# LiliMeng/network_interpretation_imagenet

Measured on NVIDIA B200. Metric: masked forward evals/sec (ResNet-101 224^2), higher is better.
Workload: dtype bf16

## Files before the change

### include/nib.h

```cpp
#ifndef NIB_H_
#define NIB_H_

#include <stddef.h>
#include <stdint.h>

#ifdef __cplusplus
extern "C" {
#endif

#define NIB_ABI_VERSION 2

enum nib_status {
  NIB_OK = 0,
  NIB_EINVAL = -1,
  NIB_ECUDA = -2,
  NIB_ENODEVICE = -3,
  NIB_ENOMEM = -4,
  NIB_ESTATE = -5,
  NIB_ENUMERIC = -6
};

int nib_abi_version(void);
const char* nib_last_error(void);
int nib_device_info(int dev, int* sm_major, int* sm_minor, int* num_sms);


enum nib_mask_mode {
  NIB_MASK_KEEP_MUL = 0,
  NIB_MASK_REMOVE_MINMAX = 1
};

enum nib_dtype { NIB_F32 = 0, NIB_BF16 = 1 };

enum nib_layout { NIB_NCHW = 0, NIB_NHWC = 1 };

typedef struct nib_mask_args {
  const float* d_img;
  const void* d_labels;
  int label_bytes;
  const uint64_t* d_sel;
  int sel_words;
  int N, C, H, W, S;
  int mode;
  const float* d_seg_minmax;
  void* d_out;
  int out_dtype;
  int layout;
  int c_stride;
  int pad_h, pad_w;
  uint8_t* d_pixel_mask;
} nib_mask_args;

int nib_segment_minmax(const float* d_img, const void* d_labels, int label_bytes,
                       int C, int H, int W, int S, float* d_seg_minmax, void* stream);

int nib_mask_synth(const nib_mask_args* args, void* stream);

int nib_mask_display_u8(const nib_mask_args* args, uint8_t* d_out, void* stream);

int nib_prep_minmax_u8(float* d_org, int C, int H, int W, uint8_t* d_u8, void* stream);


typedef struct nib_net nib_net;

enum nib_precision {
  NIB_PREC_FP32 = 0,
  NIB_PREC_BF16 = 1,
  NIB_PREC_X3 = 2,
  NIB_PREC_SPLIT = 3
};

int nib_net_create(int precision, int max_batch, nib_net** out);
int nib_net_destroy(nib_net* net);

int nib_net_add_buffer(nib_net* net, int H, int W, int C, int pad);

int nib_net_add_buffer_f32(nib_net* net, int H, int W, int C, int pad);
int nib_net_add_convert(nib_net* net, int in_buf, int out_buf);

enum nib_conv_flags {
  NIB_CONV_RELU = 1,
  NIB_CONV_PRE_BNRELU = 2
};

typedef struct nib_conv_desc {
  int in_buf, in_coff, Cin;
  int out_buf, out_coff, Cout;
  int res_buf, res_coff, res_C;
  int R, S, stride, pad;
  int flags;
} nib_conv_desc;

int nib_net_add_conv(nib_net* net, const nib_conv_desc* d, const float* h_weight,
                     const float* h_bias, const float* h_pre_scale, const float* h_pre_shift);

enum nib_pool_kind { NIB_POOL_MAX = 0, NIB_POOL_AVG = 1 };
int nib_net_add_pool(nib_net* net, int kind, int in_buf, int in_coff, int C, int out_buf,
                     int out_coff, int k, int stride, int pad,
                     const float* h_pre_scale, const float* h_pre_shift);

int nib_net_add_fc(nib_net* net, int in_buf, int Cin, int Cout, const float* h_weight,
                   const float* h_bias);

int nib_net_set_input(nib_net* net, int buf);
int nib_net_finalize(nib_net* net);

enum nib_input_layout {
  NIB_IN_NCHW_F32 = 0,
  NIB_IN_NATIVE = 1
};

int nib_net_forward(nib_net* net, const void* d_x, int x_layout, int N, float* d_logits,
                    void* stream);

int nib_net_forward_masked(nib_net* net, const nib_mask_args* args, float* d_logits, void* stream);

int nib_net_buffer_info(nib_net* net, int buf, void** d_ptr, int* H, int* W, int* C, int* pad,
                        int* dtype);
int nib_net_read_buffer_nchw(nib_net* net, int buf, int N, float* d_out, void* stream);

int nib_net_launch_counts(nib_net* net, long long* total, long long* tcgen05);
int nib_net_set_tensor_core(nib_net* net, int enable);
int nib_net_set_graph(nib_net* net, int enable);

int nib_net_profile(nib_net* net, int N, float* h_ms, int* h_kind, double* h_flops, int* h_geom,
                    int cap, int* num_ops, void* stream);

int nib_score(const float* d_logits, int N, int K, int target, int32_t* d_top1,
              float* d_target_prob, float* d_max_prob, uint8_t* d_correct, float* d_margin,
              void* stream);

int nib_score_table(const float* d_logits, int N, int K, int target, int32_t* d_top1,
                    float* d_target_prob, float* d_max_prob, uint8_t* d_correct, float* d_margin,
                    float* d_table, void* stream);

int nib_tie_compact(const float* d_margin, int N, float threshold, const uint64_t* d_sel, int words, int cap,
                    int32_t* d_idx, uint64_t* d_sel_out, int32_t* d_count, long long* d_totals, void* stream);
int nib_tie_scatter(const int32_t* d_idx, const int32_t* d_count, int cap, const int32_t* r_top1,
                    const float* r_target_prob, const float* r_max_prob, const uint8_t* r_correct,
                    int32_t* d_top1, float* d_target_prob, float* d_max_prob, uint8_t* d_correct,
                    float* d_table, void* stream);
int nib_net_set_dynamic_batch(nib_net* net, const int32_t* d_count);

typedef struct nib_comm nib_comm;
int nib_comm_unique_id(void* h_id128);
int nib_comm_init(const void* h_id128, int rank, int world, nib_comm** out);
int nib_comm_destroy(nib_comm* comm);
int nib_allgather_scores(nib_comm* comm, const float* d_local, int rows_per_rank, float* d_table, void* stream);

int nib_tc_gemm_bf16(const void* d_A, const void* d_B, float* d_C, int M, int N, int K,
                     void* stream);


int nib_gp_gram_binary(const uint64_t* d_Za, int na, const uint64_t* d_Zb, int nb, int words,
                       double length_scale, double jitter, double* d_K, int ldk, void* stream);

int nib_gp_gram_rbf(const double* d_Xa, int na, const double* d_Xb, int nb, int d,
                    double length_scale, double jitter, int same, double* d_K, int ldk,
                    void* stream);

int nib_gp_cholesky(double* d_K, int n, int ldk, int* d_info, void* stream);

int nib_gp_dgemm_sub(const double* d_A, const double* d_B, double* d_C, int M, int N, int K, void* stream);

int nib_gp_trsm(const double* d_L, int n, int ldl, double* d_B, int nrhs, int ldb, int trans,
// ... 56 lines not shown
```

### network_interpretation_imagenet_b200/_lib.py

```python
from __future__ import annotations

import ctypes as C
import os

PKG_DIR = os.path.dirname(os.path.abspath(__file__))
LIB_PATH = os.path.join(PKG_DIR, "libnib.so")

NIB_OK = 0
ABI_VERSION = 2
MASK_KEEP_MUL, MASK_REMOVE_MINMAX = 0, 1
F32, BF16 = 0, 1
NCHW, NHWC = 0, 1
PREC_FP32, PREC_BF16, PREC_X3, PREC_SPLIT = 0, 1, 2, 3
CONV_RELU, CONV_PRE_BNRELU = 1, 2
POOL_MAX, POOL_AVG = 0, 1
IN_NCHW_F32, IN_NATIVE = 0, 1


class NibError(RuntimeError):
    def __init__(self, code: int, where: str, msg: str):
        super().__init__(f"{where} failed with code {code}: {msg}")
        self.code = code


class MaskArgs(C.Structure):
    _fields_ = [
        ("d_img", C.c_void_p), ("d_labels", C.c_void_p), ("label_bytes", C.c_int),
        ("d_sel", C.c_void_p), ("sel_words", C.c_int),
        ("N", C.c_int), ("C", C.c_int), ("H", C.c_int), ("W", C.c_int), ("S", C.c_int),
        ("mode", C.c_int), ("d_seg_minmax", C.c_void_p),
        ("d_out", C.c_void_p), ("out_dtype", C.c_int), ("layout", C.c_int),
        ("c_stride", C.c_int), ("pad_h", C.c_int), ("pad_w", C.c_int),
        ("d_pixel_mask", C.c_void_p),
    ]


class ConvDesc(C.Structure):
    _fields_ = [
        ("in_buf", C.c_int), ("in_coff", C.c_int), ("Cin", C.c_int),
        ("out_buf", C.c_int), ("out_coff", C.c_int), ("Cout", C.c_int),
        ("res_buf", C.c_int), ("res_coff", C.c_int), ("res_C", C.c_int),
        ("R", C.c_int), ("S", C.c_int), ("stride", C.c_int), ("pad", C.c_int),
        ("flags", C.c_int),
    ]


_vp, _i, _d = C.c_void_p, C.c_int, C.c_double
_PROTOTYPES = {
    "nib_abi_version": (C.c_int, []),
    "nib_last_error": (C.c_char_p, []),
    "nib_device_info": (_i, [_i, C.POINTER(_i), C.POINTER(_i), C.POINTER(_i)]),
    "nib_segment_minmax": (_i, [_vp, _vp, _i, _i, _i, _i, _i, _vp, _vp]),
    "nib_mask_synth": (_i, [C.POINTER(MaskArgs), _vp]),
    "nib_mask_display_u8": (_i, [C.POINTER(MaskArgs), _vp, _vp]),
    "nib_prep_minmax_u8": (_i, [_vp, _i, _i, _i, _vp, _vp]),
    "nib_net_create": (_i, [_i, _i, C.POINTER(_vp)]),
    "nib_net_destroy": (_i, [_vp]),
    "nib_net_add_buffer": (_i, [_vp, _i, _i, _i, _i]),
    "nib_net_add_buffer_f32": (_i, [_vp, _i, _i, _i, _i]),
    "nib_net_add_convert": (_i, [_vp, _i, _i]),
    "nib_net_add_conv": (_i, [_vp, C.POINTER(ConvDesc), _vp, _vp, _vp, _vp]),
    "nib_net_add_pool": (_i, [_vp, _i, _i, _i, _i, _i, _i, _i, _i, _i, _vp, _vp]),
    "nib_net_add_fc": (_i, [_vp, _i, _i, _i, _vp, _vp]),
    "nib_net_set_input": (_i, [_vp, _i]),
    "nib_net_finalize": (_i, [_vp]),
    "nib_net_forward": (_i, [_vp, _vp, _i, _i, _vp, _vp]),
    "nib_net_forward_masked": (_i, [_vp, C.POINTER(MaskArgs), _vp, _vp]),
    "nib_net_buffer_info": (_i, [_vp, _i, C.POINTER(_vp), C.POINTER(_i), C.POINTER(_i), C.POINTER(_i),
                                 C.POINTER(_i), C.POINTER(_i)]),
    "nib_net_read_buffer_nchw": (_i, [_vp, _i, _i, _vp, _vp]),
    "nib_net_launch_counts": (_i, [_vp, C.POINTER(C.c_longlong), C.POINTER(C.c_longlong)]),
    "nib_net_set_tensor_core": (_i, [_vp, _i]),
    "nib_net_set_graph": (_i, [_vp, _i]),
    "nib_net_profile": (_i, [_vp, _i, _vp, _vp, _vp, _vp, _i, C.POINTER(_i), _vp]),
    "nib_score": (_i, [_vp, _i, _i, _i, _vp, _vp, _vp, _vp, _vp, _vp]),
    "nib_score_table": (_i, [_vp, _i, _i, _i, _vp, _vp, _vp, _vp, _vp, _vp, _vp]),
    "nib_tie_compact": (_i, [_vp, _i, C.c_float, _vp, _i, _i, _vp, _vp, _vp, _vp, _vp]),
    "nib_tie_scatter": (_i, [_vp, _vp, _i, _vp, _vp, _vp, _vp, _vp, _vp, _vp, _vp, _vp, _vp]),
    "nib_net_set_dynamic_batch": (_i, [_vp, _vp]),
    "nib_comm_unique_id": (_i, [_vp]),
    "nib_comm_init": (_i, [_vp, _i, _i, C.POINTER(_vp)]),
    "nib_comm_destroy": (_i, [_vp]),
    "nib_allgather_scores": (_i, [_vp, _vp, _i, _vp, _vp]),
    "nib_tc_gemm_bf16": (_i, [_vp, _vp, _vp, _i, _i, _i, _vp]),
    "nib_gp_gram_binary": (_i, [_vp, _i, _vp, _i, _i, _d, _d, _vp, _i, _vp]),
    "nib_gp_gram_rbf": (_i, [_vp, _i, _vp, _i, _i, _d, _d, _i, _vp, _i, _vp]),
    "nib_gp_cholesky": (_i, [_vp, _i, _i, _vp, _vp]),
    "nib_gp_trsm": (_i, [_vp, _i, _i, _vp, _i, _i, _i, _vp]),
    "nib_gp_dgemm_sub": (_i, [_vp, _vp, _vp, _i, _i, _i, _vp]),
    "nib_gp_posterior": (_i, [_vp, _i, _i, _vp, _vp, _i, _i, _d, _d, _d, _vp, _vp, _vp, _vp, _vp]),
    "nib_gp_lml": (_i, [_vp, _i, _i, _vp, _vp, C.POINTER(_d), _vp]),
    "nib_gp_lml_grad": (_i, [_vp, _vp, _vp, _vp, _i, _i, _i, _d, C.POINTER(_d), _vp]),
    "nib_gp_lml_grad_rbf": (_i, [_vp, _vp, _vp, _vp, _i, _i, _i, _d, C.POINTER(_d), _vp]),
    "nib_gp_ei": (_i, [_vp, _vp, _i, _d, _i, _vp, _vp, _vp]),
    "nib_gp_gemv_t": (_i, [_vp, _i, _i, _i, _vp, _vp, _vp]),
    "nib_gp_colsumsq": (_i, [_vp, _i, _i, _i, _vp, _vp]),
    "nib_gp_append_row": (_i, [_vp, _vp, _d, _vp, _vp, _i, _vp]),
# ... 56 lines not shown
```

### network_interpretation_imagenet_b200/classifier.py

```python
from __future__ import annotations

import ctypes as C

import numpy as np
import torch
import torch.nn as nn

from . import _lib


def _f32(t: torch.Tensor) -> np.ndarray:
    return np.ascontiguousarray(t.detach().to(torch.float32).cpu().numpy())


def fold_bn(conv_w: torch.Tensor, conv_b: torch.Tensor | None, bn: nn.BatchNorm2d | None):
    w = conv_w.detach().double()
    b = conv_b.detach().double() if conv_b is not None else torch.zeros(w.shape[0], dtype=torch.float64, device=w.device)
    if bn is not None:
        scale = bn.weight.detach().double() / torch.sqrt(bn.running_var.detach().double() + bn.eps)
        w = w * scale.view(-1, 1, 1, 1)
        b = bn.bias.detach().double() + (b - bn.running_mean.detach().double()) * scale
    elif conv_b is None:
        return w.float(), None
    return w.float(), b.float()


def bn_affine(bn: nn.BatchNorm2d):
    scale = bn.weight.detach().double() / torch.sqrt(bn.running_var.detach().double() + bn.eps)
    shift = bn.bias.detach().double() - bn.running_mean.detach().double() * scale
    return scale.float(), shift.float()


class _Builder:

    def __init__(self, precision: int, max_batch: int):
        self.lib = _lib.load()
        h = C.c_void_p()
        _lib.check(self.lib.nib_net_create(precision, max_batch, C.byref(h)), "nib_net_create")
        self.h = h
        self.shapes: dict[int, tuple[int, int, int]] = {}
        self.free: dict[tuple[int, int, int], list[int]] = {}

    def buffer(self, H, W, Cc, pad=0, pooled=True, f32=False) -> int:
        key = (H, W, Cc, bool(f32))
        if pooled and pad == 0 and self.free.get(key):
            return self.free[key].pop()
        b = (self.lib.nib_net_add_buffer_f32 if f32 else self.lib.nib_net_add_buffer)(self.h, H, W, Cc, pad)
        if b < 0:
            _lib.check(b, "nib_net_add_buffer")
        self.shapes[b] = key
        return b

    def convert(self, in_buf: int, out_buf: int):
        _lib.check(self.lib.nib_net_add_convert(self.h, in_buf, out_buf), "nib_net_add_convert")

    def release(self, b: int):
        self.free.setdefault(self.shapes[b], []).append(b)

    def conv(self, in_buf, Cin, out_buf, Cout, w, b, k, stride, pad, relu, in_coff=0, out_coff=0, res=None, res_C=0,
             pre=None):
        d = _lib.ConvDesc()
        d.in_buf, d.in_coff, d.Cin = in_buf, in_coff, Cin
        d.out_buf, d.out_coff, d.Cout = out_buf, out_coff, Cout
        d.res_buf, d.res_coff, d.res_C = (res if res is not None else -1), 0, res_C
        d.R = d.S = k
        d.stride, d.pad = stride, pad
        d.flags = (_lib.CONV_RELU if relu else 0) | (_lib.CONV_PRE_BNRELU if pre is not None else 0)
        wn = _f32(w)
        bn_ = _f32(b) if b is not None else None
        ps = _f32(pre[0]) if pre is not None else None
        pb = _f32(pre[1]) if pre is not None else None
        _lib.check(self.lib.nib_net_add_conv(self.h, C.byref(d), wn.ctypes.data,
                                             bn_.ctypes.data if bn_ is not None else None,
                                             ps.ctypes.data if ps is not None else None,
                                             pb.ctypes.data if pb is not None else None), "nib_net_add_conv")

    def pool(self, kind, in_buf, Cc, out_buf, k, stride, pad, in_coff=0, out_coff=0, pre=None):
        ps = _f32(pre[0]) if pre is not None else None
        pb = _f32(pre[1]) if pre is not None else None
        _lib.check(self.lib.nib_net_add_pool(self.h, kind, in_buf, in_coff, Cc, out_buf, out_coff, k, stride, pad,
                                             ps.ctypes.data if ps is not None else None,
                                             pb.ctypes.data if pb is not None else None), "nib_net_add_pool")

    def fc(self, in_buf, Cin, Cout, w, b):
        wn, bn_ = _f32(w), (_f32(b) if b is not None else None)
        _lib.check(self.lib.nib_net_add_fc(self.h, in_buf, Cin, Cout, wn.ctypes.data,
                                           bn_.ctypes.data if bn_ is not None else None), "nib_net_add_fc")


def _out_hw(H, k, s, p):
    return (H + 2 * p - k) // s + 1


class Classifier:

    def __init__(self, builder: _Builder, in_buf: int, in_shape, num_classes: int, precision: str, max_batch: int,
                 taps=None, arch: str = ""):
        self.lib = builder.lib
        self.h = builder.h
        self.in_buf = in_buf
        self.C, self.H, self.W = in_shape
        self.num_classes = num_classes
        self.precision = precision
        self.max_batch = max_batch
        self.taps = taps or {}
        self.arch = arch
        _lib.check(self.lib.nib_net_set_input(self.h, in_buf), "nib_net_set_input")
        _lib.check(self.lib.nib_net_finalize(self.h), "nib_net_finalize")
        ptr, H, W, Cc, pad, dt = C.c_void_p(), C.c_int(), C.c_int(), C.c_int(), C.c_int(), C.c_int()
        _lib.check(self.lib.nib_net_buffer_info(self.h, in_buf, C.byref(ptr), C.byref(H), C.byref(W), C.byref(Cc),
                                                C.byref(pad), C.byref(dt)), "nib_net_buffer_info")
        self.in_c_stride, self.in_pad = Cc.value, pad.value
        self._replicas: list["Classifier"] = []
        self._streams: list = []

    def __del__(self):
        try:
            if getattr(self, "h", None):
                self.lib.nib_net_destroy(self.h)
                self.h = None
        except Exception:
            pass

    @staticmethod
    def from_torch(module: nn.Module, input_hw=None, precision: str = "bf16", max_batch: int = 128,
                   streams: int = 1) -> "Classifier":
        c = Classifier._from_torch_one(module, input_hw, precision, max_batch)
        for _ in range(max(1, int(streams)) - 1):
            c._replicas.append(Classifier._from_torch_one(module, input_hw, precision, max_batch))
        if c._replicas:
            c._streams = [torch.cuda.Stream() for _ in range(len(c._replicas) + 1)]
        return c

    @staticmethod
    def _from_torch_one(module: nn.Module, input_hw, precision: str, max_batch: int) -> "Classifier":
        prec = {"fp32": _lib.PREC_FP32, "bf16": _lib.PREC_BF16, "x3": _lib.PREC_X3, "split": _lib.PREC_SPLIT}[precision]
        m = module.module if isinstance(module, nn.DataParallel) else module
        if hasattr(m, "layer4") and hasattr(m, "fc") and hasattr(m, "maxpool"):
            return _lower_tv_resnet(m, input_hw or (224, 224), prec, precision, max_batch)
        if _is_plain_cnn(m):
            return _lower_tv_plain(m, input_hw or (224, 224), prec, precision, max_batch)
        if precision == "split":
            raise TypeError("precision 'split' (split-bf16 tensors on the tcgen05 pair kernel) is lowered for torchvision "
                            "ResNets, VGGs and AlexNet only (every body conv needs Cin % 64 == 0 and Cout % 64 == 0); use "
                            "'x3' for this network")
        if hasattr(m, "layer3") and hasattr(m, "fc") and not hasattr(m, "layer4"):
            return _lower_resnet_cifar(m, input_hw or (32, 32), prec, precision, max_batch)
        if hasattr(m, "conv6") and hasattr(m, "fc1"):
            return _lower_mnist(m, input_hw or (28, 28), prec, precision, max_batch)
        if hasattr(m, "features") and hasattr(m, "classifier") and hasattr(m.features, "denseblock1"):
# ... 12 lines not shown

    def launch_counts(self):
        a, b = C.c_longlong(), C.c_longlong()
        _lib.check(self.lib.nib_net_launch_counts(self.h, C.byref(a), C.byref(b)), "nib_net_launch_counts")
        ra = [r.launch_counts() for r in self._replicas]
        return a.value + sum(x[0] for x in ra), b.value + sum(x[1] for x in ra)

    def _round_robin(self, N: int, launch):
        if not self._replicas:
            for i in range(0, N, self.max_batch):
                launch(self, i, min(self.max_batch, N - i))
            return
        main = torch.cuda.current_stream()
        copies = [self] + self._replicas
        used = min(len(copies), (N + self.max_batch - 1) // self.max_batch)
        for s in self._streams[:used]:
            s.wait_stream(main)
        for j, i in enumerate(range(0, N, self.max_batch)):
            k = j % len(copies)
            with torch.cuda.stream(self._streams[k]):
                launch(copies[k], i, min(self.max_batch, N - i))
        for s in self._streams[:used]:
            main.wait_stream(s)

    def forward(self, x: torch.Tensor, out: torch.Tensor | None = None) -> torch.Tensor:
        if not x.is_cuda:
            raise RuntimeError("Classifier.forward needs a CUDA tensor: this engine has no CPU path")
        x = x.to(torch.float32).contiguous()
        N = int(x.shape[0])
        if tuple(x.shape[1:]) != (self.C, self.H, self.W):
            raise ValueError(f"input {tuple(x.shape)} does not match network input {(self.C, self.H, self.W)}")
        if out is None:
            out = torch.empty(N, self.num_classes, dtype=torch.float32, device=x.device)

        def launch(c, i, n):
            _lib.check(c.lib.nib_net_forward(c.h, x[i:i + n].data_ptr(), _lib.IN_NCHW_F32, n,
                                             out[i:i + n].data_ptr(), _lib.stream_handle()), "nib_net_forward")

        self._round_robin(N, launch)
        return out

    def forward_masked(self, synth, sel_bits, mode: int, out: torch.Tensor | None = None) -> torch.Tensor:
        d_sel = synth.device_bits(sel_bits)
        N = int(d_sel.shape[0])
        if out is None:
            out = torch.empty(N, self.num_classes, dtype=torch.float32, device=d_sel.device)
        if mode == _lib.MASK_REMOVE_MINMAX:
            synth.seg_minmax()

        def launch(c, i, n):
            a = synth.mask_args(d_sel[i:i + n], mode, None, 0, 0)
            _lib.check(c.lib.nib_net_forward_masked(c.h, C.byref(a), out[i:i + n].data_ptr(), _lib.stream_handle()),
                       "nib_net_forward_masked")

        self._round_robin(N, launch)
        return out

    def profile(self, N: int):
        cap = 4096
        ms = (C.c_float * cap)()
        kind = (C.c_int * cap)()
        flops = (C.c_double * cap)()
        geom = (C.c_int * (8 * cap))()
        n = C.c_int()
        _lib.check(self.lib.nib_net_profile(self.h, N, ms, kind, flops, geom, cap, C.byref(n), _lib.stream_handle()),
                   "nib_net_profile")
        return [(ms[i], kind[i], flops[i], tuple(geom[8 * i:8 * i + 8])) for i in range(n.value)]

    def read_tap(self, name: str, N: int) -> torch.Tensor:
        buf = self.taps[name]
        H, W, Cc = C.c_int(), C.c_int(), C.c_int()
        _lib.check(self.lib.nib_net_buffer_info(self.h, buf, None, C.byref(H), C.byref(W), C.byref(Cc), None, None),
                   "nib_net_buffer_info")
        out = torch.empty(N, Cc.value, H.value, W.value, dtype=torch.float32, device="cuda")
        _lib.check(self.lib.nib_net_read_buffer_nchw(self.h, buf, N, out.data_ptr(), _lib.stream_handle()),
                   "nib_net_read_buffer_nchw")
        return out


def _in_cpad(Cin: int) -> int:
    return 4 if Cin <= 4 else Cin


def _lower_tv_resnet(m, hw, prec, precision, max_batch):
    H, W = hw
    b = _Builder(prec, max_batch)
    cin = m.conv1.in_channels
    c1 = m.conv1
    stem_tc = (precision == "bf16" and c1.kernel_size == (7, 7) and c1.stride == (2, 2) and c1.padding == (3, 3) and cin <= 8)
    split = precision == "split"
    x_in = (b.buffer(H, W, 4 if cin <= 4 else 8, pad=3, pooled=False) if stem_tc
            else b.buffer(H, W, _in_cpad(cin), pooled=False, f32=split))
    Hc, Wc = _out_hw(H, c1.kernel_size[0], c1.stride[0], c1.padding[0]), _out_hw(W, c1.kernel_size[0], c1.stride[0], c1.padding[0])
    t = b.buffer(Hc, Wc, c1.out_channels, f32=split)
    w, bias = fold_bn(c1.weight, c1.bias, m.bn1)
    b.conv(x_in, cin, t, c1.out_channels, w, bias, c1.kernel_size[0], c1.stride[0], c1.padding[0], relu=True)
    mp = m.maxpool
    k, s, p = mp.kernel_size, mp.stride, mp.padding
    Hp, Wp = _out_hw(Hc, k, s, p), _out_hw(Wc, k, s, p)
    x = b.buffer(Hp, Wp, c1.out_channels, f32=split)
    b.pool(_lib.POOL_MAX, t, c1.out_channels, x, k, s, p)
    b.release(t)
    if split:
        xs = b.buffer(Hp, Wp, c1.out_channels)
        b.convert(x, xs)
        b.release(x)
        x = xs
    Cx, Hx, Wx = c1.out_channels, Hp, Wp
    for layer in (m.layer1, m.layer2, m.layer3, m.layer4):
        for blk in layer:
            convs = [(blk.conv1, blk.bn1), (blk.conv2, blk.bn2)]
            if hasattr(blk, "conv3"):
                convs.append((blk.conv3, blk.bn3))
            if blk.downsample is not None:
                dc, dbn = blk.downsample[0], blk.downsample[1]
                Hd, Wd = _out_hw(Hx, dc.kernel_size[0], dc.stride[0], dc.padding[0]), _out_hw(Wx, dc.kernel_size[0], dc.stride[0], dc.padding[0])
                idn = b.buffer(Hd, Wd, dc.out_channels)
                w, bias = fold_bn(dc.weight, dc.bias, dbn)
                b.conv(x, Cx, idn, dc.out_channels, w, bias, dc.kernel_size[0], dc.stride[0], dc.padding[0], relu=False)
            else:
                idn = x
            cur, Cc, Hh, Ww = x, Cx, Hx, Wx
            tmp = []
            for i, (cv, bn) in enumerate(convs):
                last = i == len(convs) - 1
                Ho, Wo = _out_hw(Hh, cv.kernel_size[0], cv.stride[0], cv.padding[0]), _out_hw(Ww, cv.kernel_size[0], cv.stride[0], cv.padding[0])
                o = b.buffer(Ho, Wo, cv.out_channels)
                w, bias = fold_bn(cv.weight, cv.bias, bn)
                if last:
                    b.conv(cur, Cc, o, cv.out_channels, w, bias, cv.kernel_size[0], cv.stride[0], cv.padding[0],
                           relu=True, res=idn, res_C=cv.out_channels)
                else:
                    b.conv(cur, Cc, o, cv.out_channels, w, bias, cv.kernel_size[0], cv.stride[0], cv.padding[0], relu=True)
                    tmp.append(o)
                cur, Cc, Hh, Ww = o, cv.out_channels, Ho, Wo
            for tbuf in tmp:
                b.release(tbuf)
            if idn != x:
                b.release(idn)
            b.release(x)
            x, Cx, Hx, Wx = cur, Cc, Hh, Ww
    if split:
        xf = b.buffer(Hx, Wx, Cx, f32=True)
        b.convert(x, xf)
        x = xf
    feat = b.buffer(1, 1, Cx, f32=split)
    assert Hx == Wx, "global average pool expects a square map"
    b.pool(_lib.POOL_AVG, x, Cx, feat, Hx, Hx, 0)
    b.fc(feat, Cx, m.fc.out_features, m.fc.weight, m.fc.bias)
    return Classifier(b, x_in, (cin, H, W), m.fc.out_features, precision, max_batch, arch="tv_resnet")


def _lower_resnet_cifar(m, hw, prec, precision, max_batch):
    H, W = hw
    b = _Builder(prec, max_batch)
    cp = (lambda c: max(c, 64)) if precision == "bf16" else (lambda c: c)

    def padw(w, bias, co, ci):
        if co == w.shape[0] and ci == w.shape[1]:
            return w, bias
        wp = torch.zeros(co, ci, w.shape[2], w.shape[3], dtype=w.dtype, device=w.device)
        wp[:w.shape[0], :w.shape[1]] = w
        bp = None
        if bias is not None:
            bp = torch.zeros(co, dtype=bias.dtype, device=bias.device)
            bp[:bias.shape[0]] = bias
        return wp, bp

    x_in = b.buffer(H, W, _in_cpad(3), pooled=False)
    x = b.buffer(H, W, cp(16))
    w, bias = padw(*fold_bn(m.conv1.weight, None, m.bn1), cp(16), 3)
    b.conv(x_in, 3, x, cp(16), w, bias, 3, 1, 1, relu=True)
    Cx, Hx, Wx = 16, H, W
    for layer in (m.layer1, m.layer2, m.layer3):
        for blk in layer:
            s = blk.conv1.stride[0]
            planes = blk.conv1.out_channels
            Ho, Wo = _out_hw(Hx, 3, s, 1), _out_hw(Wx, 3, s, 1)
            t = b.buffer(Ho, Wo, cp(planes))
            w, bias = padw(*fold_bn(blk.conv1.weight, None, blk.bn1), cp(planes), cp(Cx))
            b.conv(x, cp(Cx), t, cp(planes), w, bias, 3, s, 1, relu=True)
            if blk.downsample is not None:
                ks = blk.downsample.avg.kernel_size
                ks = ks if isinstance(ks, int) else ks[0]
                idn = b.buffer(_out_hw(Hx, ks, ks, 0), _out_hw(Wx, ks, ks, 0), cp(Cx))
                b.pool(_lib.POOL_AVG, x, cp(Cx), idn, ks, ks, 0)
            else:
                idn = x
            o = b.buffer(Ho, Wo, cp(planes))
            w, bias = padw(*fold_bn(blk.conv2.weight, None, blk.bn2), cp(planes), cp(planes))
            b.conv(t, cp(planes), o, cp(planes), w, bias, 3, 1, 1, relu=True, res=idn, res_C=cp(Cx))
            b.release(t)
            if idn != x:
                b.release(idn)
            b.release(x)
            x, Cx, Hx, Wx = o, planes, Ho, Wo
    ks = m.avgpool.kernel_size
    ks = ks if isinstance(ks, int) else ks[0]
    assert _out_hw(Hx, ks, ks, 0) == 1, "AvgPool2d(8) must reduce to 1x1 (models/resnet.py:103)"
    feat = b.buffer(1, 1, cp(Cx))
    b.pool(_lib.POOL_AVG, x, cp(Cx), feat, ks, ks, 0)
    fw = m.fc.weight
    if cp(Cx) != Cx:
        fw = torch.zeros(fw.shape[0], cp(Cx), dtype=fw.dtype, device=fw.device)
        fw[:, :Cx] = m.fc.weight
    b.fc(feat, cp(Cx), m.fc.out_features, fw, m.fc.bias)
    return Classifier(b, x_in, (3, H, W), m.fc.out_features, precision, max_batch, arch="resnet_cifar")


def _lower_mnist(m, hw, prec, precision, max_batch):
    H, W = hw
    b = _Builder(prec, max_batch)
    x_in = b.buffer(H, W, _in_cpad(1), pooled=False)
    cur, Cc, Hh, Ww = x_in, 1, H, W
    taps = {}
    for name in ("conv1", "conv2", "conv3", "conv4", "conv5"):
        seq = getattr(m, name)
        cv, bn = seq[0], seq[1]
        Ho, Wo = _out_hw(Hh, 3, cv.stride[0], cv.padding[0]), _out_hw(Ww, 3, cv.stride[0], cv.padding[0])
        o = b.buffer(Ho, Wo, cv.out_channels, pooled=False)
        w, bias = fold_bn(cv.weight, cv.bias, bn)
        b.conv(cur, Cc, o, cv.out_channels, w, bias, 3, cv.stride[0], cv.padding[0], relu=True)
        cur, Cc, Hh, Ww = o, cv.out_channels, Ho, Wo
        if name == "conv2":
            taps["x0"] = o
        if name == "conv4":
            taps["x1"] = o
    cv = m.conv6
    o = b.buffer(Hh, Ww, cv.out_channels, pooled=False)
    b.conv(cur, Cc, o, cv.out_channels, cv.weight.detach().float(), cv.bias.detach().float(), 3, 1, 1, relu=False)
    taps["x2"] = o
    feat = b.buffer(1, 1, cv.out_channels)
    assert Hh == Ww
    b.pool(_lib.POOL_AVG, o, cv.out_channels, feat, Hh, Hh, 0)
    b.fc(feat, cv.out_channels, m.fc1.out_features, m.fc1.weight, m.fc1.bias)
    return Classifier(b, x_in, (1, H, W), m.fc1.out_features, precision, max_batch, taps=taps, arch="mnist")


def _dense_block(b: _Builder, layers, blk_buf, C0, H, W, Ctot):
    cur = C0
    for lyr in layers:
        n1, c1 = lyr.norm1, lyr.conv1
        has_bottleneck = hasattr(lyr, "conv2") and getattr(lyr, "conv2") is not None
        if has_bottleneck:
            n2, c2 = lyr.norm2, lyr.conv2
            mid = b.buffer(H, W, c1.out_channels)
            w, bias = fold_bn(c1.weight, None, n2)
            b.conv(blk_buf, cur, mid, c1.out_channels, w, bias, 1, 1, 0, relu=True, pre=bn_affine(n1))
            b.conv(mid, c1.out_channels, blk_buf, c2.out_channels, c2.weight.detach().float(), None, 3, 1, 1,
                   relu=False, out_coff=cur)
            b.release(mid)
            cur += c2.out_channels
        else:
            b.conv(blk_buf, cur, blk_buf, c1.out_channels, c1.weight.detach().float(), None, 3, 1, 1, relu=False,
                   out_coff=cur, pre=bn_affine(n1))
            cur += c1.out_channels
    assert cur == Ctot
    return cur


def _lower_tv_densenet(m, hw, prec, precision, max_batch):
    H, W = hw
    f = m.features
    b = _Builder(prec, max_batch)
    c0 = f.conv0
    stem_tc = (precision == "bf16" and c0.kernel_size == (7, 7) and c0.stride == (2, 2) and c0.padding == (3, 3))
    x_in = b.buffer(H, W, 4, pad=3, pooled=False) if stem_tc else b.buffer(H, W, _in_cpad(3), pooled=False)
    Hc, Wc = _out_hw(H, 7, 2, 3), _out_hw(W, 7, 2, 3)
    t = b.buffer(Hc, Wc, c0.out_channels)
    w, bias = fold_bn(c0.weight, None, f.norm0)
    b.conv(x_in, 3, t, c0.out_channels, w, bias, 7, 2, 3, relu=True)
    Hx, Wx = _out_hw(Hc, 3, 2, 1), _out_hw(Wc, 3, 2, 1)
    blocks = [getattr(f, n) for n in ("denseblock1", "denseblock2", "denseblock3", "denseblock4")]
    trans = [getattr(f, n) for n in ("transition1", "transition2", "transition3")]
    Cin = c0.out_channels
    prev, prev_is_stem = t, True
    for bi, blk in enumerate(blocks):
        layers = list(blk.children())
        growth = layers[0].conv2.out_channels
        Ctot = Cin + growth * len(layers)
        buf = b.buffer(Hx, Wx, Ctot, pooled=False)
        if prev_is_stem:
            b.pool(_lib.POOL_MAX, prev, Cin, buf, 3, 2, 1)
            b.release(prev)
        else:
            b.pool(_lib.POOL_AVG, prev, Cin, buf, 2, 2, 0)
            b.release(prev)
        _dense_block(b, layers, buf, Cin, Hx, Wx, Ctot)
        if bi < len(trans):
            tr = trans[bi]
            Co = tr.conv.out_channels
            tt = b.buffer(Hx, Wx, Co)
            b.conv(buf, Ctot, tt, Co, tr.conv.weight.detach().float(), None, 1, 1, 0, relu=False, pre=bn_affine(tr.norm))
            prev, prev_is_stem = tt, False
            Cin = Co
            Hx, Wx = Hx // 2, Wx // 2
        else:
            feat = b.buffer(1, 1, Ctot)
            assert Hx == Wx
            b.pool(_lib.POOL_AVG, buf, Ctot, feat, Hx, Hx, 0, pre=bn_affine(f.norm5))
            b.fc(feat, Ctot, m.classifier.out_features, m.classifier.weight, m.classifier.bias)
    return Classifier(b, x_in, (3, H, W), m.classifier.out_features, precision, max_batch, arch="tv_densenet")


def _lower_densenet_cifar(m, hw, prec, precision, max_batch):
    H, W = hw
    b = _Builder(prec, max_batch)
    x_in = b.buffer(H, W, _in_cpad(3), pooled=False)
    seq = list(m.blocks.children())
    Cin = m.stem.out_channels
    Hx, Wx = H, W
    prev = None
    for i in range(0, len(seq), 2):
        layers = list(seq[i].children())
        growth = (layers[0].conv2 if hasattr(layers[0], "conv2") else layers[0].conv1).out_channels
        Ctot = Cin + growth * len(layers)
        buf = b.buffer(Hx, Wx, Ctot, pooled=False)
        if prev is None:
            b.conv(x_in, 3, buf, Cin, m.stem.weight.detach().float(), None, 3, 1, 1, relu=False)
        else:
            b.pool(_lib.POOL_AVG, prev, Cin, buf, 2, 2, 0)
            b.release(prev)
        _dense_block(b, layers, buf, Cin, Hx, Wx, Ctot)
        if i + 1 < len(seq):
            tr = list(seq[i + 1].children())
            Co = tr[2].out_channels
            tt = b.buffer(Hx, Wx, Co)
            b.conv(buf, Ctot, tt, Co, tr[2].weight.detach().float(), None, 1, 1, 0, relu=False, pre=bn_affine(tr[0]))
            prev, Cin = tt, Co
            Hx, Wx = Hx // 2, Wx // 2
        else:
            feat = b.buffer(1, 1, Ctot)
            assert Hx == 8 and Wx == 8, "avg_pool2d(8) expects an 8x8 map (models/densenet.py:96)"
            b.pool(_lib.POOL_AVG, buf, Ctot, feat, 8, 8, 0, pre=bn_affine(m.norm5))
            b.fc(feat, Ctot, m.classifier.out_features, m.classifier.weight, m.classifier.bias)
    return Classifier(b, x_in, (3, H, W), m.classifier.out_features, precision, max_batch, arch="densenet_cifar")


def _is_plain_cnn(m) -> bool:
    return (isinstance(getattr(m, "features", None), nn.Sequential) and isinstance(getattr(m, "classifier", None), nn.Sequential)
            and not hasattr(m.features, "denseblock1"))


def _pair(v):
    return tuple(v) if isinstance(v, (tuple, list)) else (v, v)


def _plain_cnn_layers(m, hw, precision):
    H, W = hw
    C = None
    ops = []
    mods = list(m.features.children())
    i = 0
    while i < len(mods):
        mod = mods[i]
        if isinstance(mod, nn.Conv2d):
            k, s, p, d = _pair(mod.kernel_size), _pair(mod.stride), _pair(mod.padding), _pair(mod.dilation)
            if (mod.groups != 1 or d != (1, 1) or k[0] != k[1] or s[0] != s[1] or isinstance(mod.padding, str) or p[0] != p[1]
                    or mod.padding_mode != "zeros"):
                raise TypeError(f"unsupported Conv2d in features[{i}]: {mod} (needs groups 1, dilation 1, square kernel, "
                                "stride and zero padding)")
            if C is not None and mod.in_channels != C:
                raise TypeError(f"features[{i}]: {mod} takes {mod.in_channels} channels, the map has {C}")
            bn = None
            if i + 1 < len(mods) and isinstance(mods[i + 1], nn.BatchNorm2d):
# ... 121 lines not shown
```

### network_interpretation_imagenet_b200/csrc/conv_tc.cu

```cuda
#include "common.cuh"
#include "layers.cuh"
#include <cuda.h>
#include <string.h>
#include <stdlib.h>

namespace nib {

static constexpr int TC_BLOCK_M = 128;
static constexpr int TC_BLOCK_K = 64;
static constexpr int TC_UMMA_K = 16;
static constexpr int TC_THREADS = 192;

struct TcKernelParams {
  const float* bias;
  const __nv_bfloat16* res;
  void* out;
  int M;
  int Cout;
  int out_cstride, out_coff;
  int res_cstride, res_coff;
  int relu;
  int out_f32;
  int num_k_blocks;
  int cblocks;
// ... 412 lines not shown
                                             int c2, int c3) {
  asm volatile(
      "cp.async.bulk.tensor.4d.cta_group::2.shared::cluster.global.mbarrier::complete_tx::bytes [%0], [%1, {%3, %4, %5, %6}], [%2];"
      ::"r"(dst), "l"(reinterpret_cast<uint64_t>(tm)), "r"(leader_bar), "r"(c0), "r"(c1), "r"(c2), "r"(c3)
      : "memory");
}
__device__ __forceinline__ void tma2_load_5d(uint32_t dst, const CUtensorMap* tm, uint32_t leader_bar, int c0, int c1,
                                             int c2, int c3, int c4) {
  asm volatile(
      "cp.async.bulk.tensor.5d.cta_group::2.shared::cluster.global.mbarrier::complete_tx::bytes [%0], [%1, {%3, %4, %5, %6, %7}], [%2];"
      ::"r"(dst), "l"(reinterpret_cast<uint64_t>(tm)), "r"(leader_bar), "r"(c0), "r"(c1), "r"(c2), "r"(c3), "r"(c4)
      : "memory");
}
__device__ __forceinline__ void tma2_load_im2col_4d(uint32_t dst, const CUtensorMap* tm, uint32_t leader_bar, int c,
                                                    int w, int h, int n, uint16_t off_w, uint16_t off_h) {
  asm volatile(
      "cp.async.bulk.tensor.4d.im2col.cta_group::2.shared::cluster.global.mbarrier::complete_tx::bytes"
      " [%0], [%1, {%3, %4, %5, %6}], [%2], {%7, %8};"
      ::"r"(dst), "l"(reinterpret_cast<uint64_t>(tm)), "r"(leader_bar), "r"(c), "r"(w), "r"(h), "r"(n), "h"(off_w),
      "h"(off_h)
      : "memory");
}
__device__ __forceinline__ bool elect_one() {
  uint32_t pred;
  asm volatile(
      "{\n\t.reg .pred p;\n\t"
      "elect.sync _|p, 0xffffffff;\n\t"
      "selp.u32 %0, 1, 0, p;\n\t}"
      : "=r"(pred));
  return pred != 0;
}
__device__ __forceinline__ void named_bar_sync(int id, int nthreads) {
  asm volatile("bar.sync %0, %1;" ::"r"(id), "r"(nthreads) : "memory");
}

__device__ __forceinline__ void tmem_ld_32x32b_x64(uint32_t taddr, uint32_t (&v)[64]) {
  asm volatile(
      "tcgen05.ld.sync.aligned.32x32b.x64.b32 "
      "{%0, %1, %2, %3, %4, %5, %6, %7, %8, %9, %10, %11, %12, %13, %14, %15, "
      "%16, %17, %18, %19, %20, %21, %22, %23, %24, %25, %26, %27, %28, %29, %30, %31, "
      "%32, %33, %34, %35, %36, %37, %38, %39, %40, %41, %42, %43, %44, %45, %46, %47, "
      "%48, %49, %50, %51, %52, %53, %54, %55, %56, %57, %58, %59, %60, %61, %62, %63}, [%64];"
      : "=r"(v[0]), "=r"(v[1]), "=r"(v[2]), "=r"(v[3]), "=r"(v[4]), "=r"(v[5]), "=r"(v[6]), "=r"(v[7]),
        "=r"(v[8]), "=r"(v[9]), "=r"(v[10]), "=r"(v[11]), "=r"(v[12]), "=r"(v[13]), "=r"(v[14]), "=r"(v[15]),
        "=r"(v[16]), "=r"(v[17]), "=r"(v[18]), "=r"(v[19]), "=r"(v[20]), "=r"(v[21]), "=r"(v[22]), "=r"(v[23]),
        "=r"(v[24]), "=r"(v[25]), "=r"(v[26]), "=r"(v[27]), "=r"(v[28]), "=r"(v[29]), "=r"(v[30]), "=r"(v[31]),
        "=r"(v[32]), "=r"(v[33]), "=r"(v[34]), "=r"(v[35]), "=r"(v[36]), "=r"(v[37]), "=r"(v[38]), "=r"(v[39]),
        "=r"(v[40]), "=r"(v[41]), "=r"(v[42]), "=r"(v[43]), "=r"(v[44]), "=r"(v[45]), "=r"(v[46]), "=r"(v[47]),
        "=r"(v[48]), "=r"(v[49]), "=r"(v[50]), "=r"(v[51]), "=r"(v[52]), "=r"(v[53]), "=r"(v[54]), "=r"(v[55]),
        "=r"(v[56]), "=r"(v[57]), "=r"(v[58]), "=r"(v[59]), "=r"(v[60]), "=r"(v[61]), "=r"(v[62]), "=r"(v[63])
      : "r"(taddr)
      : "memory");
}
__device__ __forceinline__ uint64_t pack_f32x2(uint32_t lo, uint32_t hi) {
  uint64_t r;
  asm("mov.b64 %0, {%1, %2};" : "=l"(r) : "r"(lo), "r"(hi));
  return r;
}
__device__ __forceinline__ uint64_t add_f32x2(uint64_t a, uint64_t b) {
  uint64_t r;
  asm("add.rn.f32x2 %0, %1, %2;" : "=l"(r) : "l"(a), "l"(b));
  return r;
}
__device__ __forceinline__ uint32_t cvt_bf16x2(uint64_t a) {
  uint32_t lo, hi, r;
  asm("mov.b64 {%0, %1}, %2;" : "=r"(lo), "=r"(hi) : "l"(a));
  asm("cvt.rn.bf16x2.f32 %0, %1, %2;" : "=r"(r) : "f"(__uint_as_float(hi)), "f"(__uint_as_float(lo)));
  return r;
}
__device__ __forceinline__ uint32_t max_bf16x2(uint32_t a, uint32_t b) {
  uint32_t r;
  asm("max.NaN.bf16x2 %0, %1, %2;" : "=r"(r) : "r"(a), "r"(b));
  return r;
}
__device__ __forceinline__ void mbar_arrive_remote(uint32_t cluster_addr) {
  asm volatile("mbarrier.arrive.shared::cluster.b64 _, [%0];" ::"r"(cluster_addr) : "memory");
}

template <int BLOCK_N>
__host__ __device__ constexpr uint32_t make_idesc_bf16_pair() {
  return (1u << 4) | (1u << 7) | (1u << 10) | ((uint32_t)(BLOCK_N >> 3) << 17) | ((uint32_t)(256 >> 4) << 24);
}

template <int BLOCK_N, int STAGES, bool HAS_RES, bool BRES, bool SPLIT = false>
__global__ void __cluster_dims__(2, 1, 1) __launch_bounds__(TC3_THREADS_XF, 1)
conv_tc3_kernel(const __grid_constant__ CUtensorMap tmA, const __grid_constant__ CUtensorMap tmB,
                const __grid_constant__ CUtensorMap tmOut, const __grid_constant__ CUtensorMap tmOutTail,
                const __grid_constant__ CUtensorMap tmRes, const TcKernelParams p) {
  using SM = Tc3Smem<BLOCK_N, STAGES, HAS_RES, BRES, SPLIT>;
  extern __shared__ __align__(1024) uint8_t smem_raw[];
  const uint32_t smem_base = smem_u32(smem_raw);
  if ((smem_base & 1023u) != 0) {
    if (threadIdx.x == 0 && p.err_flag) atomicExch(p.err_flag, 9u);
    __trap();
  }
  const uint32_t bar_base = smem_base + SM::BAR_OFFSET;
  auto full_bar = [&](int s) { return bar_base + 8u * s; };
  auto empty_bar = [&](int s) { return bar_base + 8u * (STAGES + s); };
  auto tmem_full_bar = [&](int b) { return bar_base + 8u * (2 * STAGES + b); };
  auto tmem_empty_bar = [&](int b) { return bar_base + 8u * (2 * STAGES + 2 + b); };
  auto res_full_bar = [&](int b) { return bar_base + 8u * (2 * STAGES + 4 + b); };
  auto box_free_bar = [&](int b) { return bar_base + 8u * (2 * STAGES + 4 + SM::NBUF + b); };
  const uint32_t bres_full_bar = bar_base + 8u * (2 * STAGES + 4 + 2 * SM::NBUF);
  auto afull_bar = [&](int s) { return bar_base + 8u * (2 * STAGES + 5 + 2 * SM::NBUF + s); };
  auto xf_bar = [&](int s) { return bar_base + 8u * (3 * STAGES + 5 + 2 * SM::NBUF + s); };
  const bool xform = !BRES && !SPLIT && p.xf_scale != nullptr;
  const uint32_t tmem_slot = bar_base + 8u * SM::NUM_BARS;
  uint32_t* tmem_slot_ptr = reinterpret_cast<uint32_t*>(smem_raw + (tmem_slot - smem_u32(smem_raw)));
  auto box_addr = [&](int buf) { return smem_base + SM::BOX_OFFSET + (uint32_t)buf * SM::BOX_BYTES; };

  const int warp = threadIdx.x >> 5;
  const int lane = threadIdx.x & 31;
  const uint32_t rank = cluster_ctarank();
  const int pair = blockIdx.x >> 1;
  const int npairs = gridDim.x >> 1;
  int m_tiles_live = p.m_tiles;
  if (SPLIT && p.dyn_n != nullptr) {
    const long long live = (long long)max(*p.dyn_n, 0) * p.P * p.Q;
    const int t = (int)((live + p.tile_rows - 1) / p.tile_rows);
    if (t < m_tiles_live) m_tiles_live = t;
  }
  const int m_pairs = (m_tiles_live + 1) >> 1;
  const int total_tiles = m_pairs * p.n_tiles;
  constexpr uint32_t TMEM_COLS = 2 * BLOCK_N;
  const bool dbg_on = p.dbg != nullptr;
  long long t_acc[4] = {0, 0, 0, 0};
  long long t_loop0 = 0;
  if (dbg_on && threadIdx.x == 0) {
    unsigned long long gt;
    asm volatile("mov.u64 %0, %%globaltimer;" : "=l"(gt));
    p.dbg[(size_t)blockIdx.x * 16 + 12] = gt;
    p.dbg[(size_t)blockIdx.x * 16 + 14] = (unsigned long long)clock64();
  }
#define TC3_TIMED(slot, stmt)                                      \
  do {                                                             \
    if (dbg_on) { const long long _t = clock64(); stmt; t_acc[slot] += clock64() - _t; } \
    else { stmt; }                                                 \
  } while (0)

  if (warp == 0 && lane == 0) {
    prefetch_tmap(&tmA);
    prefetch_tmap(&tmB);
    prefetch_tmap(&tmOut);
    if (HAS_RES) prefetch_tmap(&tmRes);
    for (int s = 0; s < STAGES; ++s) {
      mbar_init(full_bar(s), 1);
      mbar_init(empty_bar(s), 1);
    }
    for (int b = 0; b < 2; ++b) {
      mbar_init(tmem_full_bar(b), 1);
      mbar_init(tmem_empty_bar(b), SM::EMPTY_ARRIVALS);
    }
    for (int b = 0; b < SM::NBUF; ++b) {
      mbar_init(res_full_bar(b), 1);
      mbar_init(box_free_bar(b), 4);
    }
    mbar_init(bres_full_bar, 1);
    for (int s2 = 0; s2 < STAGES; ++s2) {
      mbar_init(afull_bar(s2), 1);
      mbar_init(xf_bar(s2), 2 * TC3_XF_WARPS);
    }
    asm volatile("fence.mbarrier_init.release.cluster;" ::: "memory");
  }
  if (warp == 1) {
    asm volatile("tcgen05.alloc.cta_group::2.sync.aligned.shared::cta.b32 [%0], %1;" ::"r"(tmem_slot), "r"(TMEM_COLS) : "memory");
    asm volatile("tcgen05.relinquish_alloc_permit.cta_group::2.sync.aligned;" ::: "memory");
// ... 110 lines not shown
          const int ca = SPLIT ? (cb >= p.a_wrap ? cb - p.a_wrap : cb) : cb;
          const int c0 = ca * TC_BLOCK_K + p.in_coff;
          if (p.im2col == 1) {
            tma2_load_im2col_4d(a_dst, &tmA, lbar, c0, w0, h0, img, (uint16_t)tap_s, (uint16_t)tap_r);
          } else if (p.im2col == 2) {
            tma2_load_4d(a_dst, &tmA, lbar, 0, 0, h0 + kb, img);
          } else if (p.im2col == 3) {
            tma2_load_4d(a_dst, &tmA, lbar, 0, 0, h0 + 2 * kb, img);
            tma2_load_4d(a_dst + SM::A_BYTES / 2, &tmA, lbar, 0, 0, h0 + 2 * kb + 1, img);
          } else if (xform) {
            mbar_arrive_expect_tx(afull_bar(stage), (uint32_t)p.a_bytes);
            tma_load_2d(a_dst, &tmA, afull_bar(stage), c0, m0);
          } else {
            tma2_load_2d(a_dst, &tmA, lbar, c0, m0);
          }
          if (!BRES) tma2_load_2d(a_dst + SM::A_BYTES, &tmB, lbar, kb * TC_BLOCK_K, n0 + b_row0);
        }
        __syncwarp();
        if (++stage == STAGES) { stage = 0; phase ^= 1u; }
        ++kb;
        if (++cb == p.cblocks) { cb = 0; if (++tap_s == p.S) { tap_s = 0; ++tap_r; } }
      }
      if (HAS_RES) {
        issue_pending(true);
        pend_b = 0;
        pend_set = it % SM::RSETS;
        pend_par = (uint32_t)((it / SM::RSETS) & 1);
        pend_m0 = m0;
        pend_n0 = n0;
      }
    }
    if (HAS_RES) issue_pending(true);
    if (dbg_on && lane == 0) {
      unsigned long long* d = p.dbg + (size_t)blockIdx.x * 16;
      d[0] = (unsigned long long)t_acc[0]; d[1] = (unsigned long long)t_acc[1];
      d[8] = (unsigned long long)(clock64() - t_loop0);
    }
  } else if (warp == 1) {
    if (rank == 0) {
      constexpr uint32_t idesc = make_idesc_bf16_pair<BLOCK_N>();
      int stage = 0;
      uint32_t phase = 0;
      int it = 0;
      if (dbg_on) t_loop0 = clock64();
      if (BRES) mbar_wait(bres_full_bar, 0, p.err_flag, 7);
      for (int tile = pair; tile < total_tiles; tile += npairs, ++it) {
        const int ab = it & 1;
        TC3_TIMED(1, mbar_wait(tmem_empty_bar(ab), (uint32_t)(((it >> 1) & 1) ^ 1), p.err_flag, 5));
        tc_fence_after();
        const uint32_t d_tmem = tmem_base + (uint32_t)(ab * BLOCK_N);
        if (BRES && !HAS_RES && p.im2col == 4) {
          const int npb = 4 / p.halo_cb, pbuf = it % npb;
          const int st4 = 2 * p.halo_cb * pbuf;
          TC3_TIMED(0, mbar_wait(full_bar(st4), (uint32_t)((it / npb) & 1), p.err_flag, 2));
          tc_fence_after();
          if (elect_one()) {
            const uint32_t patch = smem_base + st4 * SM::STAGE_BYTES;
            const uint32_t bhb = (uint32_t)(p.halo_n * 64);
            const uint32_t idesc_h = p.halo_n == 32 ? make_idesc_bf16_pair<32>() : idesc;
#pragma unroll 1
            for (int kb = 0; kb < 9 * p.halo_cb; ++kb) {
              const int tap = p.halo_cb == 2 ? (kb >> 1) : kb, c = p.halo_cb == 2 ? (kb & 1) : 0;
              const int dy = tap / 3, dx = tap - 3 * dy;
              const uint32_t a_addr = patch + (uint32_t)(2 * c) * SM::STAGE_BYTES + (uint32_t)(dy * p.halo_wp + dx) * 128u;
              const uint64_t adesc = make_smem_desc_sw128(a_addr);
              const uint64_t bdesc = make_smem_desc_sw128(smem_base + SM::BRES_OFFSET + (uint32_t)kb * bhb);
#pragma unroll
              for (int k = 0; k < TC_BLOCK_K / TC_UMMA_K; ++k)
                umma2_bf16(d_tmem, adesc + (uint64_t)(2 * k), bdesc + (uint64_t)(2 * k), idesc_h, (kb | k) != 0);
            }
            umma2_commit_both(empty_bar(st4));
            umma2_commit_both(tmem_full_bar(ab));
          }
          __syncwarp();
          continue;
        }
        if (BRES && !HAS_RES && p.im2col == 5) {
          TC3_TIMED(0, mbar_wait(full_bar(stage), phase, p.err_flag, 2));
          tc_fence_after();
          if (elect_one()) {
            const int q0 = ((tile / p.n_tiles) % p.col_tiles) * p.tile_rows;
            const uint32_t a_addr = smem_base + stage * SM::STAGE_BYTES + 16u * (uint32_t)q0;
            const uint32_t lbo = p.halo_swap ? 128u : 16u, sbo = p.halo_swap ? 16u : 128u;
#pragma unroll 1
            for (int r = 0; r < p.raw_rows; ++r) {
              const uint32_t b_addr = smem_base + SM::BRES_OFFSET + (r >> 1) * SM::BH_BYTES + (r & 1) * (SM::BH_BYTES / 2);
#pragma unroll
              for (int ks = 0; ks < 2; ++ks) {
                const uint64_t adesc = make_smem_desc_nosw(a_addr + (uint32_t)(r * p.halo_wp) + ks * 32, lbo, sbo);
                const uint64_t bdesc = make_smem_desc_sw64(b_addr + ks * 32);
                umma2_bf16(d_tmem, adesc, bdesc, idesc, (r | ks) != 0);
              }
            }
            umma2_commit_both(empty_bar(stage));
            umma2_commit_both(tmem_full_bar(ab));
          }
          __syncwarp();
          if (++stage == STAGES) { stage = 0; phase ^= 1u; }
          continue;
        }
        for (int kk = 0; kk < p.num_k_blocks; ++kk) {
          const int kb = kk;
          TC3_TIMED(0, mbar_wait(full_bar(stage), phase, p.err_flag, 2));
          if (xform) TC3_TIMED(0, mbar_wait(xf_bar(stage), phase, p.err_flag, 8));
          tc_fence_after();
          if (elect_one()) {
            const uint32_t a_addr = smem_base + stage * SM::STAGE_BYTES;
            const uint32_t b_addr = BRES ? smem_base + SM::BRES_OFFSET + kb * SM::BH_BYTES : a_addr + SM::A_BYTES;
            if (BRES && p.im2col == 3) {
#pragma unroll
              for (int k = 0; k < TC_BLOCK_K / TC_UMMA_K; ++k) {
                const uint64_t adesc = make_smem_desc_sw64(a_addr + (k >> 1) * (SM::A_BYTES / 2) + (k & 1) * 32);
                const uint64_t bdesc = make_smem_desc_sw64(b_addr + (k >> 1) * (SM::BH_BYTES / 2) + (k & 1) * 32);
                umma2_bf16(d_tmem, adesc, bdesc, idesc, (kk | k) != 0);
              }
            } else {
              const uint64_t adesc = make_smem_desc_sw128(a_addr);
              const uint64_t bdesc = make_smem_desc_sw128(b_addr);
#pragma unroll
              for (int k = 0; k < TC_BLOCK_K / TC_UMMA_K; ++k)
                umma2_bf16(d_tmem, adesc + (uint64_t)(2 * k), bdesc + (uint64_t)(2 * k), idesc, (kk | k) != 0);
            }
            umma2_commit_both(empty_bar(stage));
            if (kk == p.num_k_blocks - 1) umma2_commit_both(tmem_full_bar(ab));
          }
          __syncwarp();
          if (++stage == STAGES) { stage = 0; phase ^= 1u; }
        }
      }
      if (dbg_on && lane == 0) {
        unsigned long long* d = p.dbg + (size_t)blockIdx.x * 16;
        d[2] = (unsigned long long)t_acc[0]; d[3] = (unsigned long long)t_acc[1];
        d[9] = (unsigned long long)(clock64() - t_loop0);
      }
    }
  } else if (warp >= 2 + 8) {
    if (xform) {
      const int t = (int)threadIdx.x - 32 * (2 + 8);
      const int cl = t & 7, rb = t >> 3;
      const uint32_t lead_xf0 = mapa_shared(xf_bar(0), 0);
      int stage = 0;
      uint32_t phase = 0;
      for (int tile = pair; tile < total_tiles; tile += npairs) {
        for (int kk = 0; kk < p.num_k_blocks; ++kk) {
          const float4 s0 = __ldg(reinterpret_cast<const float4*>(p.xf_scale + kk * TC_BLOCK_K + 8 * cl));
          const float4 s1 = __ldg(reinterpret_cast<const float4*>(p.xf_scale + kk * TC_BLOCK_K + 8 * cl + 4));
          const float4 h0 = __ldg(reinterpret_cast<const float4*>(p.xf_shift + kk * TC_BLOCK_K + 8 * cl));
          const float4 h1 = __ldg(reinterpret_cast<const float4*>(p.xf_shift + kk * TC_BLOCK_K + 8 * cl + 4));
          mbar_wait(afull_bar(stage), phase, p.err_flag, 9);
          const uint32_t a_addr = smem_base + stage * SM::STAGE_BYTES;
#pragma unroll
          for (int i = 0; i < 8; ++i) {
            const int r = rb + 16 * i;
            const uint32_t addr = a_addr + (uint32_t)r * 128u + ((uint32_t)(cl ^ (r & 7)) << 4);
            const uint4 raw = lds_v4(addr);
            const __nv_bfloat162* v = reinterpret_cast<const __nv_bfloat162*>(&raw);
            const float2 a = __bfloat1622float2(v[0]), b = __bfloat1622float2(v[1]), c = __bfloat1622float2(v[2]), d = __bfloat1622float2(v[3]);
            uint4 o;
            __nv_bfloat162 q;
            q = __floats2bfloat162_rn(fmaxf(fmaf(a.x, s0.x, h0.x), 0.f), fmaxf(fmaf(a.y, s0.y, h0.y), 0.f)); o.x = *reinterpret_cast<uint32_t*>(&q);
            q = __floats2bfloat162_rn(fmaxf(fmaf(b.x, s0.z, h0.z), 0.f), fmaxf(fmaf(b.y, s0.w, h0.w), 0.f)); o.y = *reinterpret_cast<uint32_t*>(&q);
            q = __floats2bfloat162_rn(fmaxf(fmaf(c.x, s1.x, h1.x), 0.f), fmaxf(fmaf(c.y, s1.y, h1.y), 0.f)); o.z = *reinterpret_cast<uint32_t*>(&q);
            q = __floats2bfloat162_rn(fmaxf(fmaf(d.x, s1.z, h1.z), 0.f), fmaxf(fmaf(d.y, s1.w, h1.w), 0.f)); o.w = *reinterpret_cast<uint32_t*>(&q);
            sts_v4(addr, o);
          }
          fence_async_smem();
          __syncwarp();
          if (lane == 0) mbar_arrive_remote(lead_xf0 + 8u * stage);
          if (++stage == STAGES) { stage = 0; phase ^= 1u; }
        }
      }
    }
  } else {
    const int ew = warp - 2;
    const int g = ew >> 2;
    const int quarter = warp & 3;
// ... 141 lines not shown
          uint64_t a2 = pack_f32x2(v[c * 8 + 4], v[c * 8 + 5]), a3 = pack_f32x2(v[c * 8 + 6], v[c * 8 + 7]);
          if (has_bias) {
            const uint4 b0 = lds_v4(bsrc + (uint32_t)(c * 32)), b1 = lds_v4(bsrc + (uint32_t)(c * 32 + 16));
            a0 = add_f32x2(a0, pack_f32x2(b0.x, b0.y)); a1 = add_f32x2(a1, pack_f32x2(b0.z, b0.w));
            a2 = add_f32x2(a2, pack_f32x2(b1.x, b1.y)); a3 = add_f32x2(a3, pack_f32x2(b1.z, b1.w));
          }
          if (HAS_RES) {
            const uint4 r = lds_v4(obase + ((((uint32_t)c) ^ sw) << 4));
            a0 = add_f32x2(a0, pack_f32x2(r.x << 16, r.x & 0xFFFF0000u)); a1 = add_f32x2(a1, pack_f32x2(r.y << 16, r.y & 0xFFFF0000u));
            a2 = add_f32x2(a2, pack_f32x2(r.z << 16, r.z & 0xFFFF0000u)); a3 = add_f32x2(a3, pack_f32x2(r.w << 16, r.w & 0xFFFF0000u));
          }
          o[c * 4 + 0] = max_bf16x2(cvt_bf16x2(a0), relu_floor); o[c * 4 + 1] = max_bf16x2(cvt_bf16x2(a1), relu_floor);
          o[c * 4 + 2] = max_bf16x2(cvt_bf16x2(a2), relu_floor); o[c * 4 + 3] = max_bf16x2(cvt_bf16x2(a3), relu_floor);
        }
        if (halo) {
          if (quarter == 0 && lane == 0) TC3_TIMED(2, bulk_wait_read<0>());
          TC3_TIMED(3, named_bar_sync(1 + g, 128));
          if (halo_valid) {
#pragma unroll
            for (int c = 0; c < 8; ++c)
              if (c < 4 || p.halo_n == 64)
                sts_v4(halo_base + ((((uint32_t)c) ^ halo_sw) << 4), make_uint4(o[c * 4], o[c * 4 + 1], o[c * 4 + 2], o[c * 4 + 3]));
          }
          fence_async_smem();
          TC3_TIMED(3, named_bar_sync(1 + g, 128));
          if (quarter == 0 && lane == 0) {
            tma_store_2d(&tmOutTail, box_addr(g), p.out_coff + n0, m0);
            bulk_commit();
          }
          continue;
        }
        if (!HAS_RES) {
          if (lane == 0) TC3_TIMED(2, bulk_wait_read<0>());
          __syncwarp();
        }
#pragma unroll
        for (int c = 0; c < 8; ++c)
          sts_v4(obase + ((((uint32_t)c) ^ sw) << 4), make_uint4(o[c * 4], o[c * 4 + 1], o[c * 4 + 2], o[c * 4 + 3]));
        fence_async_smem();
        __syncwarp();
        if (lane == 0) {
          if (rows_here >= 32) tma_store_2d(&tmOut, slab, p.out_coff + n0 + b * 64, m0 + quarter * 32);
          else if (rows_here > 0) tma_store_2d(&tmOutTail, slab, p.out_coff + n0 + b * 64, m0 + quarter * 32);
          bulk_commit();
          if (HAS_RES) {
            if (u > 0) {
              TC3_TIMED(2, bulk_wait_read<1>());
              mbar_arrive(box_free_bar(buf - 1));
            }
            if (u == SM::UNITS - 1) {
              TC3_TIMED(2, bulk_wait_read<0>());
              mbar_arrive(box_free_bar(buf));
            }
          }
        }
      }
    }
    if (lane == 0) bulk_wait_read<0>();
    if (dbg_on && warp == 2 && lane == 0) {
      unsigned long long* d = p.dbg + (size_t)blockIdx.x * 16;
      d[4] = (unsigned long long)t_acc[0]; d[5] = (unsigned long long)t_acc[1];
      d[6] = (unsigned long long)t_acc[2]; d[7] = (unsigned long long)t_acc[3];
      d[10] = (unsigned long long)(clock64() - t_loop0);
      d[11] = (unsigned long long)lt;
    }
    tc_fence_before();
  }
#undef TC3_TIMED
  __syncthreads();
  cluster_sync_all();
  if (warp == 1) {
    tc_fence_after();
    asm volatile("tcgen05.dealloc.cta_group::2.sync.aligned.b32 %0, %1;" ::"r"(tmem_base), "r"(TMEM_COLS) : "memory");
  }
  if (dbg_on && threadIdx.x == 0) {
    unsigned long long gt;
    asm volatile("mov.u64 %0, %%globaltimer;" : "=l"(gt));
    p.dbg[(size_t)blockIdx.x * 16 + 13] = gt;
    p.dbg[(size_t)blockIdx.x * 16 + 15] = (unsigned long long)clock64();
  }
}


struct TcFusedParams {
  const float* bias1;
  const float* bias2;
  const __nv_bfloat16* res;
  int M, m_tiles;
  int kb1;
  int nch;
  int n1;
  int relu1, relu2;
  unsigned int* err_flag;
  unsigned long long* dbg;
};

template <int N2>
struct TcFusedSmem {
  static constexpr int S1 = 4, S2 = 4;
  static constexpr int A1_BYTES = TC_BLOCK_M * TC_BLOCK_K * 2;
  static constexpr int A1_KB = 4;
  static constexpr int B1_BYTES = 64 * TC_BLOCK_K * 2;
  static constexpr int B2_BYTES = (N2 / 2) * TC_BLOCK_K * 2;
  static constexpr int BOX_BYTES = TC_BLOCK_M * 128;
  static constexpr int R1_OFFSET = A1_KB * A1_BYTES;
  static constexpr int R2_OFFSET = R1_OFFSET + S1 * B1_BYTES;
  static constexpr int STG_OFFSET = R2_OFFSET + S2 * B2_BYTES;
  static constexpr int BIAS1_OFFSET = STG_OFFSET + 4 * BOX_BYTES;
  static constexpr int BIAS2_OFFSET = BIAS1_OFFSET + 2 * 128 * 4;
  static constexpr int BAR_OFFSET = BIAS2_OFFSET + N2 * 4;
  static constexpr int NUM_BARS = 2 * S1 + 2 * S2 + 14;
  static constexpr int TOTAL = BAR_OFFSET + NUM_BARS * 8 + 16;
  static constexpr int EP2_WARPS = N2 / 16;
};

static constexpr int TCF_THREADS = 64 + 512;
template <int N2>
__global__ void __cluster_dims__(2, 1, 1) __launch_bounds__(TCF_THREADS, 1)
conv_fused_ca_kernel(const __grid_constant__ CUtensorMap tmA1, const __grid_constant__ CUtensorMap tmB1,
                     const __grid_constant__ CUtensorMap tmRes, const __grid_constant__ CUtensorMap tmY,
                     const __grid_constant__ CUtensorMap tmB2, const __grid_constant__ CUtensorMap tmOut2,
                     const TcFusedParams p) {
  using SM = TcFusedSmem<N2>;
  constexpr int S1 = SM::S1, S2 = SM::S2;
  extern __shared__ __align__(1024) uint8_t smem_raw[];
  const uint32_t smem_base = smem_u32(smem_raw);
  if ((smem_base & 1023u) != 0) {
    if (threadIdx.x == 0 && p.err_flag) atomicExch(p.err_flag, 9u);
    __trap();
  }
  const uint32_t bar_base = smem_base + SM::BAR_OFFSET;
  auto full1 = [&](int s) { return bar_base + 8u * s; };
  auto empty1 = [&](int s) { return bar_base + 8u * (S1 + s); };
  auto full2 = [&](int s) { return bar_base + 8u * (2 * S1 + s); };
  auto empty2 = [&](int s) { return bar_base + 8u * (2 * S1 + S2 + s); };
  const uint32_t bar2 = bar_base + 8u * (2 * S1 + 2 * S2);
  auto acc1_full = [&](int b) { return bar2 + 8u * b; };
  auto acc1_empty = [&](int b) { return bar2 + 8u * (2 + b); };
  auto res_full = [&](int b) { return bar2 + 8u * (4 + b); };
  auto y_ready = [&](int b) { return bar2 + 8u * (6 + b); };
  auto stage_free = [&](int b) { return bar2 + 8u * (8 + b); };
  const uint32_t acc2_full = bar2 + 8u * 10;
  const uint32_t acc2_empty = bar2 + 8u * 11;
  const uint32_t a1_full = bar2 + 8u * 12;
  const uint32_t a1_empty = bar2 + 8u * 13;
  const uint32_t tmem_slot = bar_base + 8u * SM::NUM_BARS;
  uint32_t* tmem_slot_ptr = reinterpret_cast<uint32_t*>(smem_raw + (tmem_slot - smem_base));
  auto stg = [&](int set, int box) { return smem_base + SM::STG_OFFSET + (uint32_t)(set * 2 + box) * SM::BOX_BYTES; };
  float* bias1_s = reinterpret_cast<float*>(smem_raw + SM::BIAS1_OFFSET);
  float* bias2_s = reinterpret_cast<float*>(smem_raw + SM::BIAS2_OFFSET);

  const int warp = threadIdx.x >> 5;
  const int lane = threadIdx.x & 31;
  const uint32_t rank = cluster_ctarank();
  const int pair = blockIdx.x >> 1;
  const int npairs = gridDim.x >> 1;
  const int m_pairs = (p.m_tiles + 1) >> 1;
  constexpr uint32_t TMEM_COLS = 512;
  constexpr uint32_t ACC2_COL = 256;

  if (warp == 0 && lane == 0) {
    prefetch_tmap(&tmA1); prefetch_tmap(&tmB1); prefetch_tmap(&tmRes);
    prefetch_tmap(&tmY); prefetch_tmap(&tmB2); prefetch_tmap(&tmOut2);
    for (int s = 0; s < S1; ++s) { mbar_init(full1(s), 1); mbar_init(empty1(s), 1); }
    for (int s = 0; s < S2; ++s) { mbar_init(full2(s), 1); mbar_init(empty2(s), 1); }
    for (int b = 0; b < 2; ++b) {
// ... 233 lines not shown
          }
          __syncwarp();
          if (j + 2 < p.nch) fetch_residual(use + 1u, j + 2, m0);
          else if (more_tiles) fetch_residual(use + 1u, g, m0_next);
        }
      }
      if (ep2) {
        FT(3, mbar_wait(acc2_full, (uint32_t)it & 1u, p.err_flag, 31));
        tc_fence_after();
        if (lane == 0) bulk_wait_read<0>();
        __syncwarp();
        const int col2 = G * 64;
        drain32(lane_taddr + ACC2_COL + (uint32_t)col2, bias2_s + col2, 0, false, relu2_floor);
        drain32(lane_taddr + ACC2_COL + (uint32_t)(col2 + 32), bias2_s + col2 + 32, 4, false, relu2_floor);
        tc_fence_before();
        __syncwarp();
        if (lane == 0) mbar_arrive_remote(lead_acc2_empty);
        fence_async_smem();
        __syncwarp();
        if (lane == 0) {
          tma_store_2d(&tmOut2, slab, col2, m0 + quarter * 32);
          bulk_commit();
          bulk_wait_read<0>();
          mbar_arrive(stage_free(g));
        }
        __syncwarp();
      }
      if (ep2 && more_tiles) fetch_residual((uint32_t)((it * p.nch + (p.nch - 2 + g)) >> 1) + 1u, g, m0_next);
    }
    if (lane == 0) bulk_wait_read<0>();
    tc_fence_before();
  }
#undef FT
  if (dbg_on && lane == 0 && (warp == 0 || warp == 1 || warp == 4 || warp == 8)) {
    const int role = warp == 0 ? 0 : warp == 1 ? 1 : warp == 4 ? 2 : 3;
    unsigned long long* d = p.dbg + (size_t)blockIdx.x * 32 + role * 8;
    for (int i = 0; i < 7; ++i) d[i] = (unsigned long long)t_acc[i];
    d[7] = (unsigned long long)(clock64() - t_role0);
  }
  __syncthreads();
  cluster_sync_all();
  if (warp == 1) {
    tc_fence_after();
    asm volatile("tcgen05.dealloc.cta_group::2.sync.aligned.b32 %0, %1;" ::"r"(tmem_base), "r"(TMEM_COLS) : "memory");
  }
}

typedef CUresult (*PFN_encodeTiled)(CUtensorMap*, CUtensorMapDataType, cuuint32_t, void*, const cuuint64_t*,
                                    const cuuint64_t*, const cuuint32_t*, const cuuint32_t*, CUtensorMapInterleave,
                                    CUtensorMapSwizzle, CUtensorMapL2promotion, CUtensorMapFloatOOBfill);
typedef CUresult (*PFN_encodeIm2col)(CUtensorMap*, CUtensorMapDataType, cuuint32_t, void*, const cuuint64_t*,
                                     const cuuint64_t*, const int*, const int*, cuuint32_t, cuuint32_t,
                                     const cuuint32_t*, CUtensorMapInterleave, CUtensorMapSwizzle,
                                     CUtensorMapL2promotion, CUtensorMapFloatOOBfill);
static PFN_encodeTiled g_encodeTiled = nullptr;
static PFN_encodeIm2col g_encodeIm2col = nullptr;

static int load_driver_fns() {
  if (g_encodeTiled && g_encodeIm2col) return NIB_OK;
  cudaDriverEntryPointQueryResult q;
  void* fn = nullptr;
  NIB_CUDA(cudaGetDriverEntryPoint("cuTensorMapEncodeTiled", &fn, cudaEnableDefault, &q));
  if (q != cudaDriverEntryPointSuccess || !fn) { set_error("cuTensorMapEncodeTiled not available"); return NIB_ECUDA; }
  g_encodeTiled = (PFN_encodeTiled)fn;
  fn = nullptr;
  NIB_CUDA(cudaGetDriverEntryPoint("cuTensorMapEncodeIm2col", &fn, cudaEnableDefault, &q));
  if (q != cudaDriverEntryPointSuccess || !fn) { set_error("cuTensorMapEncodeIm2col not available"); return NIB_ECUDA; }
  g_encodeIm2col = (PFN_encodeIm2col)fn;
  return NIB_OK;
}

struct TcConvPlan {
  CUtensorMap tmA, tmB, tmOut, tmRes;
  CUtensorMap tmBh;
  CUtensorMap tmOut32, tmOutTail;
  int v3;
  int split;
  int block_n, stages;
  int im2col;
  int tile_rows;
  int num_k_blocks, cblocks;
  int halo_wp, halo_r, halo_tpi, halo_cb, halo_n;
  int raw_rows, col_tiles;
  unsigned int* err_flag;
};

static unsigned int* g_err_flag = nullptr;

static int encode_2d_bf16(CUtensorMap* tm, const void* ptr, uint64_t inner, uint64_t outer, uint64_t row_bytes,
                          uint32_t box_inner, uint32_t box_outer) {
  cuuint64_t dims[2] = {inner, outer};
  cuuint64_t strides[1] = {row_bytes};
  cuuint32_t box[2] = {box_inner, box_outer};
  cuuint32_t es[2] = {1, 1};
  CUresult r = g_encodeTiled(tm, CU_TENSOR_MAP_DATA_TYPE_BFLOAT16, 2, const_cast<void*>(ptr), dims, strides, box, es,
                             CU_TENSOR_MAP_INTERLEAVE_NONE, CU_TENSOR_MAP_SWIZZLE_128B,
                             CU_TENSOR_MAP_L2_PROMOTION_L2_256B, CU_TENSOR_MAP_FLOAT_OOB_FILL_NONE);
  if (r != CUDA_SUCCESS) {
    set_error("cuTensorMapEncodeTiled failed (%d): dims=(%llu,%llu) row_bytes=%llu box=(%u,%u) ptr=%p", (int)r,
              (unsigned long long)inner, (unsigned long long)outer, (unsigned long long)row_bytes, box_inner,
              box_outer, ptr);
    return NIB_ECUDA;
  }
  return NIB_OK;
}

bool tc_conv_is_stem(const ConvParams& p) {
  return p.R == 7 && p.S == 7 && p.stride == 2 && p.pad == 3 && p.Cin <= 8 && p.in_cstride == 8 && p.in_coff == 0 &&
         p.in_halo == 3 && p.Cout % 32 == 0 && p.Q <= TC_BLOCK_M && p.out_halo == 0 && p.out_cstride % 8 == 0 &&
         p.out_coff % 8 == 0 && p.pre_scale == nullptr && p.res == nullptr && p.w_alt != nullptr &&
         (p.Win + 2 * p.in_halo) >= 2 * (p.Q - 1) + 8;
}

bool tc_conv_is_stem4(const ConvParams& p) {
  return p.R == 7 && p.S == 7 && p.stride == 2 && p.pad == 3 && p.Cin <= 4 && p.in_cstride == 4 &&
         p.in_coff == 0 && p.in_halo == 3 && p.Cout % 64 == 0 && p.Q <= TC_BLOCK_M && p.out_halo == 0 &&
         p.out_cstride % 8 == 0 && p.out_coff % 8 == 0 && p.pre_scale == nullptr && p.res == nullptr &&
         p.w_alt != nullptr && (p.Win + 2 * p.in_halo) % 2 == 0 && (p.Win + 2 * p.in_halo) >= 2 * (p.Q - 1) + 8 &&
         (p.Hin + 2 * p.in_halo) >= 2 * (p.P - 1) + 8;
}

static int raw_row_inner(int row_el) {
  for (int c = 256; c >= 8; c -= 8)
    if (row_el % c == 0 && row_el / c <= 256) return c;
  return 0;
}

static int raw3x3_col_tiles(int Q) {
  if (Q <= TC_BLOCK_M) return 1;
  for (int t = 2; Q / t >= TC_BLOCK_M / 2; ++t)
    if (Q % t == 0 && Q / t <= TC_BLOCK_M) return t;
  return 0;
}

bool tc_conv_is_raw3x3(const ConvParams& p) {
  static const bool off = getenv("NIB_TC_NO_HALO") != nullptr;
  if (off || p.split) return false;
  if (!(p.R == 3 && p.S == 3 && p.stride == 1 && p.pad == 1 && p.Cin <= 8 && p.in_cstride == 8 && p.in_coff == 0 &&
        p.in_halo == 1))
    return false;
  if (!(p.Cout == 64 || p.Cout == 128) || p.out_halo != 0 || p.out_cstride % 8 != 0 || p.out_coff % 8 != 0) return false;
  if (p.pre_scale != nullptr || p.res != nullptr || p.w_alt == nullptr || p.P != p.Hin || p.Q != p.Win) return false;
  const int t = raw3x3_col_tiles(p.Q);
  if (t == 0) return false;
  const int Wp = p.Win + 2, row_bytes = Wp * 16;
  if (3 * row_bytes + 16 > TC_BLOCK_M * TC_BLOCK_K * 2) return false;
  if (2 * row_bytes + 16 * (p.Q - p.Q / t + TC_BLOCK_M - 1) + 64 > TC_BLOCK_M * TC_BLOCK_K * 2) return false;
  return raw_row_inner(Wp * 8) > 0;
}

static int halo_rows_per_tile(int H, int Wp) {
  for (int r = TC_BLOCK_M / Wp; r >= 1; --r)
    if (H % r == 0) return r;
  return 0;
}
bool tc_conv_is_halo3x3(const ConvParams& p) {
  static const bool off = getenv("NIB_TC_NO_HALO") != nullptr;
  if (off || p.split) return false;
  if (!(p.R == 3 && p.S == 3 && p.stride == 1 && p.pad == 1)) return false;
  if (!((p.Cin == 64 && (p.Cout == 64 || p.Cout == 32)) || (p.Cin == 128 && p.Cout == 32))) return false;
  if (p.res != nullptr || p.pre_scale != nullptr || p.in_halo != 0 || p.out_halo != 0) return false;
  if (p.in_cstride % 8 != 0 || p.in_coff % 8 != 0 || p.out_cstride % 8 != 0 || p.out_coff % 8 != 0) return false;
  if (p.P != p.Hin || p.Q != p.Win) return false;
  const int Wp = p.Win + 2;
  if (Wp > 63) return false;
  const int R = halo_rows_per_tile(p.Hin, Wp);
  return R >= 1 && R * Wp >= 56;
}

bool tc_conv_supported(const ConvParams& p) {
  if (p.split) {
    if (p.Cin % TC_BLOCK_K != 0 || p.Cout % 64 != 0 || p.in_coff != 0 || p.out_coff != 0 || p.in_lo_off != p.Cin) return false;
    if (p.in_cstride != 2 * p.Cin || p.out_cstride < p.out_lo_off + p.Cout || p.out_lo_off % 64 != 0) return false;
    if (p.in_halo != 0 || p.out_halo != 0 || p.pre_scale != nullptr || p.R != p.S || p.pad > 127 || p.R > 16) return false;
    if (p.res != nullptr && (p.res_C != p.Cout || p.res_coff != 0 || p.res_lo_off % 64 != 0 || p.res_cstride < p.res_lo_off + p.Cout))
      return false;
    return true;
  }
  if (tc_conv_is_stem(p) || tc_conv_is_stem4(p) || tc_conv_is_raw3x3(p)) return true;
  if (p.Cin % TC_BLOCK_K != 0) return false;
  if (p.in_cstride % 8 != 0 || p.in_coff % 8 != 0) return false;
  if (p.Cout % 32 != 0) return false;
  if (p.out_cstride % 8 != 0 || p.out_coff % 8 != 0) return false;
  if (p.in_halo != 0 || p.out_halo != 0) return false;
  if (p.pre_scale != nullptr && !(p.pre_padded && p.R == 1 && p.S == 1 && p.stride == 1 && p.pad == 0 && p.Cout % 64 == 0 &&
                                  p.res == nullptr))
    return false;
  if (p.res != nullptr && (p.res_C != p.Cout || p.res_cstride % 8 != 0 || p.res_coff % 8 != 0)) return false;
  if (p.R != p.S) return false;
  if (p.pad > 127 || p.R > 16) return false;
  return true;
}

static int pick_block_n(int Cout) {
  if (Cout % 256 == 0) return 256;
  if (Cout % 128 == 0) return 128;
  if (Cout % 64 == 0) return 64;
  return 32;
}

static int finish_plan(TcConvPlan* plan, const ConvParams& p, int max_batch, const void* w_ptr, int K) {
  plan->v3 = 0;
  static const bool v1_only = getenv("NIB_TC_V1") != nullptr;
  if (v1_only) return NIB_OK;
  const bool bn_ok = plan->block_n == 64 || plan->block_n == 128 || plan->block_n == 256;
  if (!bn_ok || p.Cout % plan->block_n != 0) return NIB_OK;
  const uint64_t rows = (uint64_t)max_batch * p.P * p.Q;
  int rc = encode_2d_bf16(&plan->tmOut, p.out, (uint64_t)p.out_cstride, rows, (uint64_t)p.out_cstride * 2, 64,
                          (uint32_t)plan->tile_rows);
  if (rc != NIB_OK) return rc;
  if (p.res != nullptr) {
    rc = encode_2d_bf16(&plan->tmRes, p.res, (uint64_t)p.res_cstride, rows, (uint64_t)p.res_cstride * 2, 64, TC_BLOCK_M);
    if (rc != NIB_OK) return rc;
  } else {
    plan->tmRes = plan->tmOut;
  }
  rc = encode_2d_bf16(&plan->tmBh, w_ptr, (uint64_t)K, (uint64_t)p.Cout, (uint64_t)K * 2, TC_BLOCK_K,
                      (uint32_t)(plan->block_n / 2));
  if (rc != NIB_OK) return rc;
  rc = encode_2d_bf16(&plan->tmOut32, p.out, (uint64_t)p.out_cstride, rows, (uint64_t)p.out_cstride * 2, 64, 32);
  if (rc != NIB_OK) return rc;
  const int tail = plan->tile_rows % 32;
  rc = encode_2d_bf16(&plan->tmOutTail, p.out, (uint64_t)p.out_cstride, rows, (uint64_t)p.out_cstride * 2, 64,
                      (uint32_t)(tail ? tail : 32));
  if (rc != NIB_OK) return rc;
  plan->v3 = 1;
  return NIB_OK;
}

int tc_conv_plan_create(const ConvParams& p, int max_batch, TcConvPlan** out) {
  int rc = load_driver_fns();
  if (rc != NIB_OK) return rc;
  if (!g_err_flag) {
    NIB_CUDA(cudaMalloc(&g_err_flag, sizeof(unsigned int)));
    NIB_CUDA(cudaMemset(g_err_flag, 0, sizeof(unsigned int)));
  }
  TcConvPlan* plan = new TcConvPlan();
  memset(plan, 0, sizeof(*plan));
  plan->err_flag = g_err_flag;
  plan->block_n = pick_block_n(p.Cout);
  plan->tile_rows = TC_BLOCK_M;
  if (tc_conv_is_stem4(p)) {
    plan->im2col = 3;
    plan->cblocks = 1;
    plan->num_k_blocks = 4;
    plan->tile_rows = p.Q;
    const int Hp = p.Hin + 6, Wp = p.Win + 6;
    int inner = 0;
    {
      static const bool off = getenv("NIB_TC_NO_HALO") != nullptr;
      if (!off && 6 * Wp * 8 + 16 * 127 + 64 <= 16384) inner = raw_row_inner(Wp * 4);
    }
    if (inner > 0) {
      plan->im2col = 5;
      plan->raw_rows = 7;
      plan->col_tiles = 1;
      plan->halo_wp = Wp * 8;
      cuuint64_t dims[4] = {(cuuint64_t)inner, (cuuint64_t)(Wp * 4 / inner), (cuuint64_t)Hp, (cuuint64_t)max_batch};
      cuuint64_t strides[3] = {(cuuint64_t)inner * 2, (cuuint64_t)Wp * 8, (cuuint64_t)Hp * Wp * 8};
      cuuint32_t box[4] = {(cuuint32_t)inner, (cuuint32_t)(Wp * 4 / inner), 7, 1};
      cuuint32_t es[4] = {1, 1, 1, 1};
      CUresult r = g_encodeTiled(&plan->tmA, CU_TENSOR_MAP_DATA_TYPE_BFLOAT16, 4, const_cast<void*>(p.in), dims, strides,
                                 box, es, CU_TENSOR_MAP_INTERLEAVE_NONE, CU_TENSOR_MAP_SWIZZLE_NONE,
                                 CU_TENSOR_MAP_L2_PROMOTION_L2_256B, CU_TENSOR_MAP_FLOAT_OOB_FILL_NONE);
      if (r != CUDA_SUCCESS) {
        set_error("cuTensorMapEncodeTiled (stem, raw rows) failed (%d)", (int)r);
        delete plan;
        return NIB_ECUDA;
      }
    } else {
      cuuint64_t dims[4] = {32, (cuuint64_t)p.Q, (cuuint64_t)Hp, (cuuint64_t)max_batch};
      cuuint64_t strides[3] = {16, (cuuint64_t)Wp * 8, (cuuint64_t)Hp * Wp * 8};
      cuuint32_t box[4] = {32, (cuuint32_t)p.Q, 1, 1};
      cuuint32_t es[4] = {1, 1, 1, 1};
      CUresult r = g_encodeTiled(&plan->tmA, CU_TENSOR_MAP_DATA_TYPE_BFLOAT16, 4, const_cast<void*>(p.in), dims, strides,
                                 box, es, CU_TENSOR_MAP_INTERLEAVE_NONE, CU_TENSOR_MAP_SWIZZLE_64B,
                                 CU_TENSOR_MAP_L2_PROMOTION_L2_256B, CU_TENSOR_MAP_FLOAT_OOB_FILL_NONE);
      if (r != CUDA_SUCCESS) {
        set_error("cuTensorMapEncodeTiled (stem, 4-channel rows, 64B swizzle) failed (%d)", (int)r);
        delete plan;
        return NIB_ECUDA;
      }
    }
    rc = finish_plan(plan, p, max_batch, p.w_alt, 4 * 64);
    if (rc != NIB_OK) { delete plan; return rc; }
    {
      cuuint64_t dims[2] = {256, (cuuint64_t)p.Cout};
      cuuint64_t strides[1] = {256 * 2};
      cuuint32_t box[2] = {32, (cuuint32_t)(plan->block_n / 2)};
      cuuint32_t es[2] = {1, 1};
      CUresult r = g_encodeTiled(&plan->tmBh, CU_TENSOR_MAP_DATA_TYPE_BFLOAT16, 2, const_cast<void*>(p.w_alt), dims, strides,
                                 box, es, CU_TENSOR_MAP_INTERLEAVE_NONE, CU_TENSOR_MAP_SWIZZLE_64B,
                                 CU_TENSOR_MAP_L2_PROMOTION_L2_256B, CU_TENSOR_MAP_FLOAT_OOB_FILL_NONE);
      if (r != CUDA_SUCCESS) {
        set_error("cuTensorMapEncodeTiled (stem weights, 64B swizzle) failed (%d)", (int)r);
        delete plan;
        return NIB_ECUDA;
      }
    }
    plan->tmB = plan->tmBh;
    *out = plan;
    return NIB_OK;
  }
  if (tc_conv_is_raw3x3(p)) {
    const int Hp = p.Hin + 2, Wp = p.Win + 2, row_el = Wp * 8, inner = raw_row_inner(row_el);
    plan->im2col = 5;
    plan->raw_rows = 3;
    plan->col_tiles = raw3x3_col_tiles(p.Q);
    plan->cblocks = 1;
    plan->num_k_blocks = 2;
    plan->tile_rows = p.Q / plan->col_tiles;
    plan->halo_wp = Wp * 16;
    {
      cuuint64_t dims[4] = {(cuuint64_t)inner, (cuuint64_t)(row_el / inner), (cuuint64_t)Hp, (cuuint64_t)max_batch};
      cuuint64_t strides[3] = {(cuuint64_t)inner * 2, (cuuint64_t)Wp * 16, (cuuint64_t)Hp * Wp * 16};
      cuuint32_t box[4] = {(cuuint32_t)inner, (cuuint32_t)(row_el / inner), 3, 1};
      cuuint32_t es[4] = {1, 1, 1, 1};
      CUresult r = g_encodeTiled(&plan->tmA, CU_TENSOR_MAP_DATA_TYPE_BFLOAT16, 4, const_cast<void*>(p.in), dims, strides,
                                 box, es, CU_TENSOR_MAP_INTERLEAVE_NONE, CU_TENSOR_MAP_SWIZZLE_NONE,
                                 CU_TENSOR_MAP_L2_PROMOTION_L2_256B, CU_TENSOR_MAP_FLOAT_OOB_FILL_NONE);
      if (r != CUDA_SUCCESS) {
        set_error("cuTensorMapEncodeTiled (3x3, raw rows) failed (%d)", (int)r);
        delete plan;
        return NIB_ECUDA;
      }
    }
    rc = finish_plan(plan, p, max_batch, p.w_alt, 2 * 64);
    if (rc != NIB_OK) { delete plan; return rc; }
    if (!plan->v3) { set_error("tc_conv_plan_create: the 3x3 raw-row mode needs the CTA-pair kernel"); delete plan; return NIB_EINVAL; }
    {
      cuuint64_t dims[2] = {128, (cuuint64_t)p.Cout};
      cuuint64_t strides[1] = {128 * 2};
      cuuint32_t box[2] = {32, (cuuint32_t)(plan->block_n / 2)};
      cuuint32_t es[2] = {1, 1};
      CUresult r = g_encodeTiled(&plan->tmBh, CU_TENSOR_MAP_DATA_TYPE_BFLOAT16, 2, const_cast<void*>(p.w_alt), dims, strides,
                                 box, es, CU_TENSOR_MAP_INTERLEAVE_NONE, CU_TENSOR_MAP_SWIZZLE_64B,
                                 CU_TENSOR_MAP_L2_PROMOTION_L2_256B, CU_TENSOR_MAP_FLOAT_OOB_FILL_NONE);
      if (r != CUDA_SUCCESS) {
        set_error("cuTensorMapEncodeTiled (3x3 raw-row weights, 64B swizzle) failed (%d)", (int)r);
        delete plan;
        return NIB_ECUDA;
      }
    }
    plan->tmB = plan->tmBh;
    *out = plan;
    return NIB_OK;
  }
  if (tc_conv_is_stem(p)) {
    plan->im2col = 2;
    plan->cblocks = 1;
    plan->num_k_blocks = 7;
    plan->tile_rows = p.Q;
    rc = encode_2d_bf16(&plan->tmB, p.w_alt, 7 * 64, (uint64_t)p.Cout, 7 * 64 * 2, TC_BLOCK_K, plan->block_n);
    if (rc != NIB_OK) { delete plan; return rc; }
    const int Hp = p.Hin + 6, Wp = p.Win + 6;
    cuuint64_t dims[4] = {64, (cuuint64_t)p.Q, (cuuint64_t)Hp, (cuuint64_t)max_batch};
    cuuint64_t strides[3] = {32, (cuuint64_t)Wp * 16, (cuuint64_t)Hp * Wp * 16};
    cuuint32_t box[4] = {64, (cuuint32_t)p.Q, 1, 1};
    cuuint32_t es[4] = {1, 1, 1, 1};
    CUresult r = g_encodeTiled(&plan->tmA, CU_TENSOR_MAP_DATA_TYPE_BFLOAT16, 4, const_cast<void*>(p.in), dims, strides,
                               box, es, CU_TENSOR_MAP_INTERLEAVE_NONE, CU_TENSOR_MAP_SWIZZLE_128B,
                               CU_TENSOR_MAP_L2_PROMOTION_L2_256B, CU_TENSOR_MAP_FLOAT_OOB_FILL_NONE);
    if (r != CUDA_SUCCESS) {
      set_error("cuTensorMapEncodeTiled (stem, overlapping windows) failed (%d)", (int)r);
      delete plan;
      return NIB_ECUDA;
    }
    rc = finish_plan(plan, p, max_batch, p.w_alt, 7 * 64);
    if (rc != NIB_OK) { delete plan; return rc; }
    *out = plan;
    return NIB_OK;
  }
  if (tc_conv_is_halo3x3(p)) {
    const int Wp = p.Win + 2, R = halo_rows_per_tile(p.Hin, Wp);
    plan->im2col = 4;
    plan->cblocks = p.Cin / 64;
    plan->num_k_blocks = 9 * plan->cblocks;
    plan->tile_rows = R * p.Win;
    plan->halo_wp = Wp; plan->halo_r = R; plan->halo_tpi = p.Hin / R;
    plan->halo_cb = plan->cblocks; plan->halo_n = p.Cout;
    plan->block_n = 64;
    const int Kh = 9 * p.Cin;
// ... 262 lines not shown
  NIB_CUDA(cudaLaunchKernelEx(&cfg, conv_tc3_kernel<BLOCK_N, STAGES, HAS_RES, BRES, SPLIT>, plan->tmA, plan->tmBh, plan->tmOut32,
                              plan->tmOutTail, plan->tmRes, kp));
  return NIB_OK;
}

static int tc_dispatch(const TcConvPlan* plan, const TcKernelParams& kp, int tiles, cudaStream_t st) {
  if (plan->split) {
    const bool res = kp.res != nullptr;
    if (!plan->v3 || kp.out_f32) { set_error("tc_dispatch: split mode needs the CTA-pair kernel"); return NIB_EINVAL; }
    if (plan->block_n == 256) return res ? launch_tc3<256, 3, true, false, true>(plan, kp, st) : launch_tc3<256, 6, false, false, true>(plan, kp, st);
    if (plan->block_n == 128) return res ? launch_tc3<128, 4, true, false, true>(plan, kp, st) : launch_tc3<128, 8, false, false, true>(plan, kp, st);
    return res ? launch_tc3<64, 8, true, false, true>(plan, kp, st) : launch_tc3<64, 9, false, false, true>(plan, kp, st);
  }
  if (plan->v3 && !kp.out_f32) {
    const bool res = kp.res != nullptr;
    if (plan->im2col == 4) return launch_tc3<64, 9, false, true>(plan, kp, st);
    if (plan->im2col == 5 && plan->block_n == 128) return launch_tc3<128, 6, false, true>(plan, kp, st);
    if (plan->block_n == 256) return res ? launch_tc3<256, 5, true>(plan, kp, st) : launch_tc3<256, 6, false>(plan, kp, st);
    if (plan->block_n == 128) return res ? launch_tc3<128, 6, true>(plan, kp, st) : launch_tc3<128, 8, false>(plan, kp, st);
    if (plan->block_n == 64 && !res && kp.n_tiles == 1 && kp.num_k_blocks <= TC3_BRES_KBLOCKS)
      return launch_tc3<64, 9, false, true>(plan, kp, st);
    if (plan->block_n == 64) return res ? launch_tc3<64, 9, true>(plan, kp, st) : launch_tc3<64, 9, false>(plan, kp, st);
  }
  switch (plan->block_n) {
    case 32:  return launch_tc<32, 4>(plan, kp, tiles, st);
    case 64:  return launch_tc<64, 4>(plan, kp, tiles, st);
    case 128: return launch_tc<128, 3>(plan, kp, tiles, st);
    case 256: return launch_tc<256, 4>(plan, kp, tiles, st);
  }
  set_error("tc_dispatch: bad block_n %d", plan->block_n);
  return NIB_EINVAL;
}

static int tc_launch_debug(const TcConvPlan* plan, TcKernelParams kp, const ConvParams& p, int tiles, cudaStream_t st) {
  static unsigned long long* d_dbg = nullptr;
  const int nslots = 160 * 16;
  if (!d_dbg) NIB_CUDA(cudaMalloc(&d_dbg, nslots * sizeof(unsigned long long)));
  NIB_CUDA(cudaMemsetAsync(d_dbg, 0, nslots * sizeof(unsigned long long), st));
  kp.dbg = d_dbg;
  cudaEvent_t e0, e1;
  cudaEventCreate(&e0); cudaEventCreate(&e1);
  cudaEventRecord(e0, st);
  int rc = tc_dispatch(plan, kp, tiles, st);
  cudaEventRecord(e1, st);
  if (rc != NIB_OK) return rc;
  NIB_CUDA(cudaStreamSynchronize(st));
  float ms = 0.f;
  cudaEventElapsedTime(&ms, e0, e1);
  cudaEventDestroy(e0); cudaEventDestroy(e1);
  static unsigned long long h[160 * 16];
  NIB_CUDA(cudaMemcpy(h, d_dbg, sizeof(h), cudaMemcpyDeviceToHost));
  int clk_khz = 1965000;
  cudaDeviceGetAttribute(&clk_khz, cudaDevAttrClockRate, 0);
  const double us = 1e3 / (double)clk_khz;
  double a[16] = {0};
  int nc = 0;
  unsigned long long g0 = ~0ull, g1 = 0, g0max = 0, g1min = ~0ull;
  double mhz = 0, loop_max = 0;
  for (int c = 0; c < 148; ++c) {
    if (h[c * 16 + 8] == 0) continue;
    ++nc;
    for (int j = 0; j < 12; ++j) a[j] += (double)h[c * 16 + j];
    const unsigned long long e = h[c * 16 + 12], x = h[c * 16 + 13];
    if (e < g0) g0 = e;
    if (e > g0max) g0max = e;
    if (x > g1) g1 = x;
    if (x < g1min) g1min = x;
    if (x > e) mhz += (double)(h[c * 16 + 15] - h[c * 16 + 14]) / (double)(x - e) * 1e3;
    if ((double)h[c * 16 + 10] > loop_max) loop_max = (double)h[c * 16 + 10];
  }
  fprintf(stderr, "[tc3t] in-kernel span %.1f us (first entry -> last exit), entry skew %.1f us, exit skew %.1f us, SM clock %.0f MHz, "
          "max epi loop %.1f us\n", (g1 - g0) / 1e3, (g0max - g0) / 1e3, (g1 - g1min) / 1e3, mhz / (nc ? nc : 1), loop_max * us);
  if (nc == 0) nc = 1;
  for (int j = 0; j < 16; ++j) a[j] = a[j] / nc * us;
  fprintf(stderr,
          "[tc3] %dx%d %d->%d k%d s%d res%d bn%d M=%d tiles/cta=%.1f  %.1f us | prod: loop %.1f wait_empty %.1f wait_box %.1f"
          " | mma(x2): loop %.1f wait_full %.1f wait_tmem %.1f | epi: loop %.1f wait_tmem_full %.1f wait_res %.1f"
          " store_drain %.1f bar %.1f\n",
          p.P, p.Q, p.Cin, p.Cout, p.R, p.stride, p.res != nullptr, plan->block_n, p.M, a[11], ms * 1e3, a[8], a[0], a[1],
          2 * a[9], 2 * a[2], 2 * a[3], a[10], a[4], a[5], a[6], a[7]);
  return NIB_OK;
}

int tc_conv_launch(const TcConvPlan* plan, const ConvParams& p, cudaStream_t st) {
  TcKernelParams kp;
  memset(&kp, 0, sizeof(kp));
  kp.bias = p.bias;
  kp.res = reinterpret_cast<const __nv_bfloat16*>(p.res);
  kp.out = p.out;
  kp.M = p.M;
  kp.Cout = p.Cout;
  kp.out_cstride = p.out_cstride;
  kp.out_coff = p.out_coff;
  kp.res_cstride = p.res_cstride;
  kp.res_coff = p.res_coff;
  kp.relu = p.relu;
  kp.out_f32 = 0;
  kp.num_k_blocks = plan->num_k_blocks;
  kp.cblocks = plan->cblocks;
  kp.S = p.S;
  kp.im2col = plan->im2col;
  kp.P = p.P;
  kp.Q = p.Q;
  kp.stride = p.stride;
  kp.pad = p.pad;
  kp.in_coff = p.in_coff;
  kp.n_tiles = ceil_div(p.Cout, plan->block_n);
  kp.err_flag = plan->err_flag;
  kp.tile_rows = plan->tile_rows;
  kp.a_bytes = plan->tile_rows * TC_BLOCK_K * 2;
  kp.m_tiles = ceil_div(p.M, plan->tile_rows);
  kp.a_wrap = plan->split ? 2 * p.Cin / TC_BLOCK_K : plan->cblocks;
  kp.lo_off_out = p.out_lo_off;
  kp.lo_off_res = p.res_lo_off;
  kp.dyn_n = plan->split ? p.dyn_n : nullptr;
  if (p.pre_scale != nullptr) {
    if (!(p.pre_padded && plan->im2col == 0 && plan->v3 && !plan->split)) {
      set_error("tc_conv_launch: a pre-activation conv reached a tensor path without the transform role");
      return NIB_EINVAL;
    }
    kp.xf_scale = p.pre_scale;
    kp.xf_shift = p.pre_shift;
  }
  if (plan->im2col == 4) {
    kp.n_tiles = 1;
    kp.halo_cb = plan->halo_cb; kp.halo_n = plan->halo_n;
    kp.halo_wp = plan->halo_wp; kp.halo_r = plan->halo_r; kp.halo_tpi = plan->halo_tpi;
    kp.a_bytes = (plan->halo_r + 2) * plan->halo_wp * 128;
  }
  if (plan->im2col == 5) {
    static const bool swap = getenv("NIB_TC_STEM_SWAP") != nullptr;
    kp.halo_wp = plan->halo_wp;
    kp.halo_swap = swap ? 1 : 0;
    kp.raw_rows = plan->raw_rows;
    kp.col_tiles = plan->col_tiles;
    kp.a_bytes = plan->raw_rows * plan->halo_wp;
    const int rows = p.M / p.Q;
    kp.m_tiles = (rows + 1) / 2 * 2 * plan->col_tiles;
  }
  const int tiles = kp.m_tiles * kp.n_tiles;
  static const bool dbg = getenv("NIB_TC_DBG") != nullptr;
  if (dbg && plan->v3) return tc_launch_debug(plan, kp, p, tiles, st);
  return tc_dispatch(plan, kp, tiles, st);
}

}

extern "C" int nib_tc_gemm_bf16(const void* d_A, const void* d_B, float* d_C, int M, int N, int K, void* stream) {
  NIB_DEVICE_OR_FAIL();
  using namespace nib;
  NIB_REQUIRE(d_A && d_B && d_C, "nib_tc_gemm_bf16: null pointer");
  NIB_REQUIRE(M > 0 && N > 0 && K > 0 && K % 64 == 0 && N % 32 == 0, "nib_tc_gemm_bf16: need K%%64==0, N%%32==0");
  int rc = load_driver_fns();
  if (rc != NIB_OK) return rc;
  if (!g_err_flag) {
    NIB_CUDA(cudaMalloc(&g_err_flag, sizeof(unsigned int)));
    NIB_CUDA(cudaMemset(g_err_flag, 0, sizeof(unsigned int)));
  }
  TcConvPlan plan;
  memset(&plan, 0, sizeof(plan));
  plan.err_flag = g_err_flag;
  plan.block_n = pick_block_n(N);
  plan.cblocks = K / TC_BLOCK_K;
  plan.num_k_blocks = plan.cblocks;
  plan.im2col = 0;
  rc = encode_2d_bf16(&plan.tmB, d_B, (uint64_t)K, (uint64_t)N, (uint64_t)K * 2, TC_BLOCK_K, plan.block_n);
  if (rc != NIB_OK) return rc;
// ... 21 lines not shown
```

### network_interpretation_imagenet_b200/csrc/layers.cuh

```cuda
#pragma once
#include "common.cuh"

namespace nib {

struct ConvParams {
  const void* in;
  const void* w;
  const void* w_alt;
  const float* bias;
  const void* res;
  void* out;
  const float* pre_scale;
  const float* pre_shift;
  int pre_padded;
  int M;
  int Hin, Win, Cin, in_cstride, in_coff, in_halo;
  int P, Q, Cout, out_cstride, out_coff, out_halo;
  int res_cstride, res_coff, res_C;
  int R, S, stride, pad;
  int relu;
  const int* dyn_n;
  int split;
  int in_lo_off, out_lo_off, res_lo_off;
};

struct PoolParams {
  const void* in;
  void* out;
  const float* pre_scale;
  const float* pre_shift;
  int kind, N, Hin, Win, C, in_cstride, in_coff;
  int P, Q, out_cstride, out_coff;
  int k, stride, pad;
  const int* dyn_n;
};

int launch_conv_simt(const ConvParams& p, bool bf16, cudaStream_t st);
bool conv_x3_supported(const ConvParams& p);
int launch_conv_x3(const ConvParams& p, const void* w_hi, const void* w_lo, cudaStream_t st);
int launch_pool(const PoolParams& p, bool bf16, cudaStream_t st);
bool fc_x2_supported(int Cin, int feat_stride);
int launch_fc_x2(const void* feat, int feat_stride, const void* w_hi, const void* w_lo, const float* b, int N, int Cin,
                 int Cout, float* logits, const int* dyn_n, cudaStream_t st);
int launch_fc(const void* feat, int feat_stride, bool bf16, const float* w, const float* b, int N, int Cin,
              int Cout, float* logits, const int* dyn_n, cudaStream_t st);
int launch_bnrelu_pack(const void* x, int in_cstride, int in_coff, int Cin, int Cpad, const float* scale,
                       const float* shift, void* y, long long M, cudaStream_t st);
int launch_nchw_to_nhwc(const float* x, int N, int C, int H, int W, void* out, int cs, int halo, bool bf16,
                        cudaStream_t st);
int launch_nhwc_to_nchw(const void* in, int N, int C, int H, int W, int cs, int halo, bool bf16, float* out,
                        cudaStream_t st);
int launch_split_convert(const void* in, void* out, long long M, int C, bool to_split, const int* dyn_n, int rows_per_image,
                         cudaStream_t st);
int mask_synth_impl(const nib_mask_args* a, cudaStream_t st, bool skip_halo, const int* dyn_n = nullptr);

struct TcConvPlan;

bool tc_conv_supported(const ConvParams& p);
int tc_conv_plan_create(const ConvParams& p, int max_batch, TcConvPlan** out);
void tc_conv_plan_destroy(TcConvPlan* plan);
int tc_conv_plan_block_n(const TcConvPlan* plan);
int tc_conv_launch(const TcConvPlan* plan, const ConvParams& p, cudaStream_t st);

struct TcFusedPlan;
bool tc_fuse_supported(const ConvParams& c, const ConvParams& a);
int tc_fused_plan_create(const ConvParams& c, const ConvParams& a, int max_batch, TcFusedPlan** out);
void tc_fused_plan_destroy(TcFusedPlan* plan);
int tc_fused_launch(const TcFusedPlan* plan, const ConvParams& c, const ConvParams& a, cudaStream_t st);

}
```

### network_interpretation_imagenet_b200/csrc/net.cu

```cuda
#include "common.cuh"
#include "layers.cuh"
#include <vector>
#include <map>
#include <string.h>

using namespace nib;

static constexpr size_t NIB_X3_MAX_K = 16384;

enum BufKind { BUF_F32 = 0, BUF_BF16 = 1, BUF_SPLIT = 2 };

struct NetBuffer {
  int H, W, C, pad;
  int kind;
  void* ptr;
  size_t elems_per_image;
  int phys_c() const { return kind == BUF_SPLIT ? 2 * C : C; }
  size_t esize() const { return kind == BUF_F32 ? 4 : 2; }
};

struct NetOp {
  int kind;
  nib_conv_desc cd;
  void* d_w;
// ... 88 lines not shown
}

int nib_net_destroy(nib_net* net) {
  if (!net) return NIB_OK;
  for (auto& g : net->graphs) cudaGraphExecDestroy(g.second.exec);
  for (auto& b : net->bufs)
    if (b.ptr) cudaFree(b.ptr);
  if (net->pack_scratch) cudaFree(net->pack_scratch);
  if (net->graph_logits) cudaFree(net->graph_logits);
  for (auto& o : net->ops) {
    if (o.d_w) cudaFree(o.d_w);
    if (o.d_w_pack) cudaFree(o.d_w_pack);
    if (o.d_w_alt) cudaFree(o.d_w_alt);
    if (o.d_w_hi) cudaFree(o.d_w_hi);
    if (o.d_w_lo) cudaFree(o.d_w_lo);
    if (o.d_bias) cudaFree(o.d_bias);
    if (o.d_pre_scale) cudaFree(o.d_pre_scale);
    if (o.d_pre_scale_pad) cudaFree(o.d_pre_scale_pad);
    if (o.d_pre_shift_pad) cudaFree(o.d_pre_shift_pad);
    if (o.d_pre_shift) cudaFree(o.d_pre_shift);
    if (o.plan) tc_conv_plan_destroy(o.plan);
    if (o.fplan) tc_fused_plan_destroy(o.fplan);
  }
  delete net;
  return NIB_OK;
}

static int add_buffer_kind(nib_net* net, int H, int W, int C, int pad, int kind) {
  NIB_REQUIRE(net && !net->finalized, "nib_net_add_buffer: bad handle/state");
  NIB_REQUIRE(H > 0 && W > 0 && C > 0 && pad >= 0, "nib_net_add_buffer: bad geometry");
  NetBuffer b;
  b.H = H; b.W = W; b.C = C; b.pad = pad;
  b.kind = kind;
  b.elems_per_image = (size_t)(H + 2 * pad) * (W + 2 * pad) * b.phys_c();
  size_t bytes = b.elems_per_image * net->max_batch * b.esize();
  NIB_CUDA(cudaMalloc(&b.ptr, bytes + 256));
  NIB_CUDA(cudaMemset(b.ptr, 0, bytes + 256));
  net->bufs.push_back(b);
  return (int)net->bufs.size() - 1;
}

int nib_net_add_buffer(nib_net* net, int H, int W, int C, int pad) {
  NIB_REQUIRE(net != nullptr, "nib_net_add_buffer: null handle");
  return add_buffer_kind(net, H, W, C, pad, net->bf16 ? BUF_BF16 : net->split ? BUF_SPLIT : BUF_F32);
}

int nib_net_add_buffer_f32(nib_net* net, int H, int W, int C, int pad) {
  NIB_REQUIRE(net != nullptr, "nib_net_add_buffer_f32: null handle");
  NIB_REQUIRE(!net->bf16, "nib_net_add_buffer_f32: bf16 networks have bf16 buffers only");
  return add_buffer_kind(net, H, W, C, pad, BUF_F32);
}

int nib_net_add_convert(nib_net* net, int in_buf, int out_buf) {
  NIB_REQUIRE(net && !net->finalized && net->split, "nib_net_add_convert: needs an unfinalized NIB_PREC_SPLIT network");
  const int nb = (int)net->bufs.size();
  NIB_REQUIRE(in_buf >= 0 && in_buf < nb && out_buf >= 0 && out_buf < nb, "nib_net_add_convert: bad buffer id");
  const NetBuffer& bi = net->bufs[in_buf];
  const NetBuffer& bo = net->bufs[out_buf];
  NIB_REQUIRE(bi.H == bo.H && bi.W == bo.W && bi.C == bo.C && bi.pad == 0 && bo.pad == 0, "nib_net_add_convert: geometry mismatch");
  NIB_REQUIRE((bi.kind == BUF_F32 && bo.kind == BUF_SPLIT) || (bi.kind == BUF_SPLIT && bo.kind == BUF_F32),
              "nib_net_add_convert: one side must be fp32, the other split");
  NetOp op;
  memset(&op, 0, sizeof(op));
  op.kind = 3;
  op.in_buf = in_buf;
  op.out_buf = out_buf;
  net->ops.push_back(op);
  return NIB_OK;
}

int nib_net_add_conv(nib_net* net, const nib_conv_desc* d, const float* h_weight, const float* h_bias,
                     const float* h_pre_scale, const float* h_pre_shift) {
  NIB_REQUIRE(net && !net->finalized && d && h_weight, "nib_net_add_conv: bad handle/state/args");
  const int nb = (int)net->bufs.size();
  NIB_REQUIRE(d->in_buf >= 0 && d->in_buf < nb && d->out_buf >= 0 && d->out_buf < nb, "nib_net_add_conv: bad buffer id");
  NIB_REQUIRE(d->res_buf < nb, "nib_net_add_conv: bad residual buffer id");
  const NetBuffer& bi = net->bufs[d->in_buf];
  const NetBuffer& bo = net->bufs[d->out_buf];
  NIB_REQUIRE(d->in_coff >= 0 && d->in_coff + d->Cin <= bi.C, "nib_net_add_conv: input channel slice out of range");
  NIB_REQUIRE(d->out_coff >= 0 && d->out_coff + d->Cout <= bo.C, "nib_net_add_conv: output channel slice out of range");
  NIB_REQUIRE(d->R > 0 && d->S > 0 && d->stride > 0 && d->pad >= 0, "nib_net_add_conv: bad filter geometry");
  const int P = (bi.H + 2 * d->pad - d->R) / d->stride + 1;
  const int Q = (bi.W + 2 * d->pad - d->S) / d->stride + 1;
  NIB_REQUIRE(P == bo.H && Q == bo.W, "nib_net_add_conv: output buffer is %dx%d but conv produces %dx%d", bo.H, bo.W, P, Q);
  NIB_REQUIRE(bo.pad == 0, "nib_net_add_conv: output buffers with halo are not supported");
  if (d->res_buf >= 0) {
    const NetBuffer& br = net->bufs[d->res_buf];
    NIB_REQUIRE(br.H == bo.H && br.W == bo.W && br.pad == 0, "nib_net_add_conv: residual geometry mismatch");
    NIB_REQUIRE(d->res_C > 0 && d->res_C <= d->Cout && d->res_coff + d->res_C <= br.C, "nib_net_add_conv: residual channels out of range");
  }
  if (d->flags & NIB_CONV_PRE_BNRELU) NIB_REQUIRE(h_pre_scale && h_pre_shift, "nib_net_add_conv: PRE_BNRELU needs scale/shift");

  NetOp op;
  memset(&op, 0, sizeof(op));
  op.kind = 0;
  op.cd = *d;
  NIB_REQUIRE(bi.kind == bo.kind, "nib_net_add_conv: input and output buffers must have the same kind (use nib_net_add_convert)");
  if (d->res_buf >= 0) NIB_REQUIRE(net->bufs[d->res_buf].kind == bo.kind, "nib_net_add_conv: residual buffer kind mismatch");
  const bool split_op = bi.kind == BUF_SPLIT;
  const size_t K = (size_t)d->R * d->S * d->Cin;
  const size_t nel = K * d->Cout;
  std::vector<float> krsc(nel);
  for (int co = 0; co < d->Cout; ++co)
    for (int c = 0; c < d->Cin; ++c)
      for (int r = 0; r < d->R; ++r)
        for (int s = 0; s < d->S; ++s)
          krsc[(((size_t)co * d->R + r) * d->S + s) * d->Cin + c] =
              h_weight[(((size_t)co * d->Cin + c) * d->R + r) * d->S + s];
  if (split_op) {
    const size_t taps = (size_t)d->R * d->S;
    std::vector<uint16_t> hb(nel * 3);
    for (int co = 0; co < d->Cout; ++co)
      for (size_t t = 0; t < taps; ++t)
        for (int c = 0; c < d->Cin; ++c) {
          const float w = krsc[((size_t)co * taps + t) * d->Cin + c];
          const uint16_t hi = f32_to_bf16_rn(w);
          uint32_t u = (uint32_t)hi << 16;
          float hf;
          memcpy(&hf, &u, 4);
          const uint16_t lo = f32_to_bf16_rn(w - hf);
          const size_t base = ((size_t)co * taps + t) * 3 * d->Cin;
          hb[base + c] = hi;
          hb[base + d->Cin + c] = hi;
          hb[base + 2 * (size_t)d->Cin + c] = lo;
        }
    NIB_CUDA(cudaMalloc(&op.d_w, hb.size() * 2 + 256));
    NIB_CUDA(cudaMemcpy(op.d_w, hb.data(), hb.size() * 2, cudaMemcpyHostToDevice));
  } else if (net->bf16) {
    std::vector<uint16_t> hb(nel);
    for (size_t i = 0; i < nel; ++i) hb[i] = f32_to_bf16_rn(krsc[i]);
    NIB_CUDA(cudaMalloc(&op.d_w, nel * 2 + 256));
    NIB_CUDA(cudaMemcpy(op.d_w, hb.data(), nel * 2, cudaMemcpyHostToDevice));
  } else {
    NIB_CUDA(cudaMalloc(&op.d_w, nel * 4 + 256));
    NIB_CUDA(cudaMemcpy(op.d_w, krsc.data(), nel * 4, cudaMemcpyHostToDevice));
    if (net->x3 && d->Cin % 16 == 0 && K <= NIB_X3_MAX_K) {
      std::vector<uint16_t> hi(nel), lo(nel);
      for (size_t i = 0; i < nel; ++i) {
        hi[i] = f32_to_bf16_rn(krsc[i]);
        uint32_t u = (uint32_t)hi[i] << 16;
        float hf;
        memcpy(&hf, &u, 4);
        lo[i] = f32_to_bf16_rn(krsc[i] - hf);
      }
      NIB_CUDA(cudaMalloc(&op.d_w_hi, nel * 2 + 256));
      NIB_CUDA(cudaMalloc(&op.d_w_lo, nel * 2 + 256));
      NIB_CUDA(cudaMemcpy(op.d_w_hi, hi.data(), nel * 2, cudaMemcpyHostToDevice));
      NIB_CUDA(cudaMemcpy(op.d_w_lo, lo.data(), nel * 2, cudaMemcpyHostToDevice));
    }
  }
  if (net->bf16 && d->R == 7 && d->S == 7 && d->stride == 2 && d->pad == 3 && d->Cin <= 4 && bi.C == 4 && bi.pad == 3) {
    std::vector<uint16_t> hb((size_t)d->Cout * 4 * 64, 0);
    for (int co = 0; co < d->Cout; ++co)
      for (int r = 0; r < 7; ++r)
        for (int s = 0; s < 7; ++s)
          for (int c = 0; c < d->Cin; ++c)
            hb[((size_t)co * 8 + r) * 32 + s * 4 + c] =
                f32_to_bf16_rn(h_weight[(((size_t)co * d->Cin + c) * 7 + r) * 7 + s]);
    NIB_CUDA(cudaMalloc(&op.d_w_alt, hb.size() * 2 + 256));
    NIB_CUDA(cudaMemcpy(op.d_w_alt, hb.data(), hb.size() * 2, cudaMemcpyHostToDevice));
  }
  if (net->bf16 && d->R == 7 && d->S == 7 && d->stride == 2 && d->pad == 3 && d->Cin <= 8 && bi.C == 8 && bi.pad == 3) {
    std::vector<uint16_t> hb((size_t)d->Cout * 7 * 64, 0);
    for (int co = 0; co < d->Cout; ++co)
      for (int r = 0; r < 7; ++r)
        for (int s = 0; s < 7; ++s)
          for (int c = 0; c < d->Cin; ++c)
// ... 59 lines not shown
  NIB_REQUIRE(P == bo.H && Q == bo.W, "nib_net_add_pool: output buffer is %dx%d but pool produces %dx%d", bo.H, bo.W, P, Q);
  NetOp op;
  memset(&op, 0, sizeof(op));
  op.kind = 1;
  op.pool_kind = kind; op.k = k; op.stride = stride; op.pad = pad; op.C = C;
  op.in_buf = in_buf; op.in_coff = in_coff; op.out_buf = out_buf; op.out_coff = out_coff;
  int rc = upload_floats(h_pre_scale, C, &op.d_pre_scale);
  if (rc != NIB_OK) return rc;
  rc = upload_floats(h_pre_shift, C, &op.d_pre_shift);
  if (rc != NIB_OK) return rc;
  net->ops.push_back(op);
  return NIB_OK;
}

int nib_net_add_fc(nib_net* net, int in_buf, int Cin, int Cout, const float* h_weight, const float* h_bias) {
  NIB_REQUIRE(net && !net->finalized && h_weight, "nib_net_add_fc: bad handle/state/args");
  NIB_REQUIRE(in_buf >= 0 && in_buf < (int)net->bufs.size(), "nib_net_add_fc: bad buffer id");
  const NetBuffer& bi = net->bufs[in_buf];
  NIB_REQUIRE(bi.H == 1 && bi.W == 1 && bi.C >= Cin, "nib_net_add_fc: input must be a 1x1xC feature buffer");
  NIB_REQUIRE(bi.kind != BUF_SPLIT, "nib_net_add_fc: the feature buffer must be fp32 or bf16");
  NetOp op;
  memset(&op, 0, sizeof(op));
  op.kind = 2;
  op.fc_in = in_buf; op.fc_cin = Cin; op.fc_cout = Cout;
  float* w = nullptr;
  int rc = upload_floats(h_weight, (size_t)Cin * Cout, &w);
  if (rc != NIB_OK) return rc;
  op.d_w = w;
  rc = upload_floats(h_bias, Cout, &op.d_bias);
  if (rc != NIB_OK) return rc;
  if (bi.kind == BUF_BF16 && fc_x2_supported(Cin, bi.C)) {
    const size_t nel = (size_t)Cin * Cout;
    std::vector<uint16_t> hi(nel), lo(nel);
    for (size_t i = 0; i < nel; ++i) {
      hi[i] = f32_to_bf16_rn(h_weight[i]);
      uint32_t u = (uint32_t)hi[i] << 16;
      float hf;
      memcpy(&hf, &u, 4);
      lo[i] = f32_to_bf16_rn(h_weight[i] - hf);
    }
    NIB_CUDA(cudaMalloc(&op.d_w_hi, nel * 2 + 256));
    NIB_CUDA(cudaMalloc(&op.d_w_lo, nel * 2 + 256));
    NIB_CUDA(cudaMemcpy(op.d_w_hi, hi.data(), nel * 2, cudaMemcpyHostToDevice));
    NIB_CUDA(cudaMemcpy(op.d_w_lo, lo.data(), nel * 2, cudaMemcpyHostToDevice));
  }
  net->ops.push_back(op);
  net->num_classes = Cout;
  return NIB_OK;
}

int nib_net_set_input(nib_net* net, int buf) {
  NIB_REQUIRE(net && buf >= 0 && buf < (int)net->bufs.size(), "nib_net_set_input: bad buffer id");
  net->input_buf = buf;
  return NIB_OK;
}

static void fill_conv_params(const nib_net* net, const NetOp& op, int N, ConvParams* p) {
  const nib_conv_desc& d = op.cd;
  const NetBuffer& bi = net->bufs[d.in_buf];
  const NetBuffer& bo = net->bufs[d.out_buf];
  memset(p, 0, sizeof(*p));
  p->in = bi.ptr;
  p->w = op.d_w;
  p->w_alt = op.d_w_alt;
  p->bias = op.d_bias;
  p->out = bo.ptr;
  p->pre_scale = op.d_pre_scale;
  p->pre_shift = op.d_pre_shift;
  p->Hin = bi.H; p->Win = bi.W; p->Cin = d.Cin; p->in_cstride = bi.phys_c(); p->in_coff = d.in_coff; p->in_halo = bi.pad;
  p->P = bo.H; p->Q = bo.W; p->Cout = d.Cout; p->out_cstride = bo.phys_c(); p->out_coff = d.out_coff; p->out_halo = bo.pad;
  p->split = bi.kind == BUF_SPLIT ? 1 : 0;
  p->in_lo_off = bi.C;
  p->out_lo_off = bo.C;
  p->M = N * bo.H * bo.W;
  if (d.res_buf >= 0) {
    const NetBuffer& br = net->bufs[d.res_buf];
    p->res = br.ptr;
    p->res_cstride = br.phys_c(); p->res_coff = d.res_coff; p->res_C = d.res_C;
    p->res_lo_off = br.C;
  }
  p->R = d.R; p->S = d.S; p->stride = d.stride; p->pad = d.pad;
  p->relu = (d.flags & NIB_CONV_RELU) ? 1 : 0;
  p->dyn_n = net->dyn_n;
}

static void fill_xform_conv_params(const nib_net* net, const NetOp& op, int N, ConvParams* p) {
  fill_conv_params(net, op, N, p);
  p->w = op.d_w_pack;
  p->pre_scale = op.d_pre_scale_pad;
  p->pre_shift = op.d_pre_shift_pad;
  p->pre_padded = 1;
  p->Cin = op.pack_cin;
}

static void fill_packed_conv_params(const nib_net* net, const NetOp& op, int N, ConvParams* p) {
  fill_conv_params(net, op, N, p);
  p->in = net->pack_scratch;
  p->w = op.d_w_pack;
  p->pre_scale = nullptr;
  p->pre_shift = nullptr;
  p->Cin = op.pack_cin;
  p->in_cstride = op.pack_cin;
  p->in_coff = 0;
}

int nib_net_finalize(nib_net* net) {
  NIB_REQUIRE(net && !net->finalized, "nib_net_finalize: bad handle/state");
  NIB_REQUIRE(net->input_buf >= 0, "nib_net_finalize: input buffer not set");
  NIB_REQUIRE(!net->ops.empty() && net->ops.back().kind == 2, "nib_net_finalize: the last op must be the fc layer");
  if (net->split) {
    for (auto& op : net->ops) {
      if (op.kind != 0 || net->bufs[op.cd.in_buf].kind != BUF_SPLIT) continue;
      ConvParams p;
      fill_conv_params(net, op, net->max_batch, &p);
      NIB_REQUIRE(tc_conv_supported(p), "nib_net_finalize: a conv on split tensors needs Cin %% 64 == 0, Cout %% 64 == 0, whole-buffer channel ranges (Cin=%d Cout=%d)", p.Cin, p.Cout);
      int rc = tc_conv_plan_create(p, net->max_batch, &op.plan);
      if (rc != NIB_OK) return rc;
    }
  }
  if (net->bf16) {
    static const bool no_xform = getenv("NIB_TC_NO_XFORM") != nullptr;
    for (auto& op : net->ops) {
      if (op.kind != 0 || op.pack_cin == 0) continue;
      if (!no_xform && op.d_pre_scale_pad) {
        ConvParams px;
        fill_xform_conv_params(net, op, net->max_batch, &px);
        if (tc_conv_supported(px)) { op.xform = 1; continue; }
      }
      const NetBuffer& bi = net->bufs[op.cd.in_buf];
      const size_t need = (size_t)net->max_batch * bi.H * bi.W * op.pack_cin * 2;
      if (need > net->pack_scratch_bytes) net->pack_scratch_bytes = need;
    }
    if (net->pack_scratch_bytes) NIB_CUDA(cudaMalloc(&net->pack_scratch, net->pack_scratch_bytes + 256));
    for (auto& op : net->ops) {
      if (op.kind != 0) continue;
      ConvParams p;
      if (op.xform) {
        fill_xform_conv_params(net, op, net->max_batch, &p);
        int rc = tc_conv_plan_create(p, net->max_batch, &op.plan);
        if (rc != NIB_OK) return rc;
        continue;
      }
      if (op.pack_cin) {
        fill_packed_conv_params(net, op, net->max_batch, &p);
        if (tc_conv_supported(p)) {
          int rc = tc_conv_plan_create(p, net->max_batch, &op.plan);
          if (rc != NIB_OK) return rc;
        } else {
          op.pack_cin = 0;
        }
        continue;
      }
      fill_conv_params(net, op, net->max_batch, &p);
      if (tc_conv_supported(p)) {
        int rc = tc_conv_plan_create(p, net->max_batch, &op.plan);
        if (rc != NIB_OK) {
          if (op.d_w_alt == nullptr) return rc;
          op.plan = nullptr;
        }
      }
    }
  }
  if (net->bf16) {
    for (size_t i = 0; i + 1 < net->ops.size(); ++i) {
      NetOp& c = net->ops[i];
      NetOp& a = net->ops[i + 1];
      if (c.kind != 0 || a.kind != 0 || !c.plan || !a.plan || c.pack_cin || a.pack_cin || c.fused_skip) continue;
      ConvParams pc, pa;
      fill_conv_params(net, c, net->max_batch, &pc);
      fill_conv_params(net, a, net->max_batch, &pa);
      if (!tc_fuse_supported(pc, pa)) continue;
      int rc = tc_fused_plan_create(pc, pa, net->max_batch, &c.fplan);
      if (rc != NIB_OK) return rc;
      c.next_cd = a.cd;
      c.next_w = a.d_w;
      c.next_bias = a.d_bias;
      a.fused_skip = true;
    }
  }
  net->finalized = true;
  return NIB_OK;
}

static int run_ops(nib_net* net, int N, float* d_logits, cudaStream_t st) {
  for (auto& op : net->ops) {
    if (op.kind == 0) {
      if (op.fused_skip && net->use_tc) continue;
      ConvParams p;
      fill_conv_params(net, op, N, &p);
      int rc;
      if (op.fplan && net->use_tc) {
        NetOp nx = op;
        nx.cd = op.next_cd;
        nx.d_w = op.next_w;
        nx.d_bias = op.next_bias;
        ConvParams pa;
        fill_conv_params(net, nx, N, &pa);
        rc = tc_fused_launch(op.fplan, p, pa, st);
        net->tc_launches++;
      } else if (op.plan && net->use_tc && op.xform) {
        fill_xform_conv_params(net, op, N, &p);
        rc = tc_conv_launch(op.plan, p, st);
        net->tc_launches++;
      } else if (op.plan && net->use_tc && op.pack_cin) {
        const NetBuffer& bi = net->bufs[op.cd.in_buf];
        rc = launch_bnrelu_pack(bi.ptr, bi.C, op.cd.in_coff, op.cd.Cin, op.pack_cin, op.d_pre_scale, op.d_pre_shift,
                                net->pack_scratch, (long long)N * bi.H * bi.W, st);
        net->launches++;
        if (rc != NIB_OK) return rc;
        fill_packed_conv_params(net, op, N, &p);
        rc = tc_conv_launch(op.plan, p, st);
        net->tc_launches++;
      } else if (op.plan && (net->use_tc || net->split)) {
        rc = tc_conv_launch(op.plan, p, st);
        net->tc_launches++;
      } else if (net->x3 && op.d_w_hi && conv_x3_supported(p)) {
        rc = launch_conv_x3(p, op.d_w_hi, op.d_w_lo, st);
        net->x3_launches++;
      } else {
        rc = launch_conv_simt(p, net->bf16, st);
      }
      net->launches++;
      if (rc != NIB_OK) return rc;
    } else if (op.kind == 3) {
      const NetBuffer& bi = net->bufs[op.in_buf];
      const NetBuffer& bo = net->bufs[op.out_buf];
      int rc = launch_split_convert(bi.ptr, bo.ptr, (long long)N * bi.H * bi.W, bi.C, bi.kind == BUF_F32, net->dyn_n, bi.H * bi.W, st);
      net->launches++;
      if (rc != NIB_OK) return rc;
    } else if (op.kind == 1) {
      const NetBuffer& bi = net->bufs[op.in_buf];
      const NetBuffer& bo = net->bufs[op.out_buf];
      PoolParams p;
      memset(&p, 0, sizeof(p));
      p.in = bi.ptr; p.out = bo.ptr;
      p.pre_scale = op.d_pre_scale; p.pre_shift = op.d_pre_shift;
      p.kind = op.pool_kind; p.N = N; p.Hin = bi.H; p.Win = bi.W; p.C = op.C;
      p.in_cstride = bi.C; p.in_coff = op.in_coff;
      p.P = bo.H; p.Q = bo.W; p.out_cstride = bo.C; p.out_coff = op.out_coff;
      p.k = op.k; p.stride = op.stride; p.pad = op.pad;
      p.dyn_n = net->dyn_n;
      int rc = launch_pool(p, bi.kind == BUF_BF16, st);
      net->launches++;
      if (rc != NIB_OK) return rc;
    } else {
      const NetBuffer& bi = net->bufs[op.fc_in];
      static const bool fc_simt = getenv("NIB_FC_SIMT") != nullptr;
      int rc = (op.d_w_hi && !fc_simt)
                   ? launch_fc_x2(bi.ptr, bi.C, op.d_w_hi, op.d_w_lo, op.d_bias, N, op.fc_cin, op.fc_cout, d_logits, net->dyn_n, st)
                   : launch_fc(bi.ptr, bi.C, bi.kind == BUF_BF16, (const float*)op.d_w, op.d_bias, N, op.fc_cin, op.fc_cout,
                               d_logits, net->dyn_n, st);
      net->launches++;
      if (rc != NIB_OK) return rc;
    }
  }
  return NIB_OK;
}

static int stage_input(nib_net* net, const void* d_x, int x_layout, int N, cudaStream_t st) {
  const NetBuffer& bi = net->bufs[net->input_buf];
  NIB_REQUIRE(bi.kind != BUF_SPLIT, "nib_net_forward: the input buffer of a split network must be fp32 (nib_net_add_buffer_f32)");
  if (x_layout == NIB_IN_NCHW_F32) {
    int C = bi.C;
    for (auto& op : net->ops)
      if (op.kind == 0 && op.cd.in_buf == net->input_buf) { C = op.cd.Cin; break; }
    int rc = launch_nchw_to_nhwc((const float*)d_x, N, C, bi.H, bi.W, bi.ptr, bi.C, bi.pad, net->bf16, st);
    net->launches++;
    return rc;
  }
  if (d_x != bi.ptr)
    NIB_CUDA(cudaMemcpyAsync(bi.ptr, d_x, bi.elems_per_image * N * elem_size(net), cudaMemcpyDeviceToDevice, st));
  return NIB_OK;
}

int nib_net_forward(nib_net* net, const void* d_x, int x_layout, int N, float* d_logits, void* stream) {
  NIB_DEVICE_OR_FAIL();
  NIB_REQUIRE(net && net->finalized, "nib_net_forward: network not finalized");
  NIB_REQUIRE(d_x && d_logits, "nib_net_forward: null pointer");
  NIB_REQUIRE(N > 0 && N <= net->max_batch, "nib_net_forward: N=%d outside (0, max_batch=%d]", N, net->max_batch);
  NIB_REQUIRE(x_layout == NIB_IN_NCHW_F32 || x_layout == NIB_IN_NATIVE, "nib_net_forward: bad x_layout");
  cudaStream_t st = (cudaStream_t)stream;
  if (!net->use_graph) {
    int rc = stage_input(net, d_x, x_layout, N, st);
    if (rc != NIB_OK) return rc;
    return run_ops(net, N, d_logits, st);
  }
  int rc = stage_input(net, d_x, x_layout, N, st);
  if (rc != NIB_OK) return rc;
  if (!net->graph_logits)
    NIB_CUDA(cudaMalloc(&net->graph_logits, sizeof(float) * (size_t)net->max_batch * (net->num_classes > 0 ? net->num_classes : 1)));
  auto it = net->graphs.find(N);
  if (it == net->graphs.end()) {
    if (net->graphs.size() >= nib_net::kMaxGraphs) {
      for (auto& g : net->graphs) cudaGraphExecDestroy(g.second.exec);
      net->graphs.clear();
    }
    cudaStream_t cap;
    NIB_CUDA(cudaStreamCreateWithFlags(&cap, cudaStreamNonBlocking));
    const long long l0 = net->launches, t0 = net->tc_launches;
    NIB_CUDA(cudaStreamBeginCapture(cap, cudaStreamCaptureModeThreadLocal));
    rc = run_ops(net, N, net->graph_logits, cap);
    cudaGraph_t graph = nullptr;
    cudaError_t ce = cudaStreamEndCapture(cap, &graph);
    if (rc != NIB_OK || ce != cudaSuccess) {
      if (graph) cudaGraphDestroy(graph);
      cudaStreamDestroy(cap);
      if (rc == NIB_OK) { set_error("cudaStreamEndCapture: %s", cudaGetErrorString(ce)); rc = NIB_ECUDA; }
      return rc;
    }
    nib_net::GraphVal val;
    val.launches = net->launches - l0;
    val.tc_launches = net->tc_launches - t0;
    net->launches = l0;
    net->tc_launches = t0;
    NIB_CUDA(cudaGraphInstantiate(&val.exec, graph, 0));
    cudaGraphDestroy(graph);
    cudaStreamDestroy(cap);
    it = net->graphs.insert({N, val}).first;
  }
  NIB_CUDA(cudaGraphLaunch(it->second.exec, st));
  NIB_CUDA(cudaMemcpyAsync(d_logits, net->graph_logits, sizeof(float) * (size_t)N * net->num_classes, cudaMemcpyDeviceToDevice, st));
  net->launches += it->second.launches;
  net->tc_launches += it->second.tc_launches;
  return NIB_OK;
}

int nib_net_profile(nib_net* net, int N, float* h_ms, int* h_kind, double* h_flops, int* h_geom, int cap,
                    int* num_ops, void* stream) {
  NIB_DEVICE_OR_FAIL();
  NIB_REQUIRE(net && net->finalized && h_ms && h_kind && h_flops && num_ops, "nib_net_profile: bad arguments");
  NIB_REQUIRE(N > 0 && N <= net->max_batch, "nib_net_profile: bad N");
  const int nops = (int)net->ops.size();
  NIB_REQUIRE(cap >= nops, "nib_net_profile: cap=%d < %d ops", cap, nops);
  cudaStream_t st = (cudaStream_t)stream;
  std::vector<cudaEvent_t> ev(nops + 1);
  for (auto& e : ev) NIB_CUDA(cudaEventCreate(&e));
  float* d_logits = nullptr;
  NIB_CUDA(cudaMalloc(&d_logits, sizeof(float) * (size_t)N * (net->num_classes > 0 ? net->num_classes : 1)));
  std::vector<NetOp> all;
  all.swap(net->ops);
  int rc = NIB_OK;
  for (int i = 0; i < nops && rc == NIB_OK; ++i) {
    cudaEventRecord(ev[i], st);
    net->ops.assign(1, all[i]);
    rc = run_ops(net, N, d_logits, st);
  }
  cudaEventRecord(ev[nops], st);
  net->ops.swap(all);
  cudaError_t ce = cudaStreamSynchronize(st);
  if (rc == NIB_OK && ce != cudaSuccess) { set_error("nib_net_profile: %s", cudaGetErrorString(ce)); rc = NIB_ECUDA; }
  for (int i = 0; i < nops && rc == NIB_OK; ++i) {
    cudaEventElapsedTime(&h_ms[i], ev[i], ev[i + 1]);
    const NetOp& op = net->ops[i];
    if (op.kind == 0) {
      const NetBuffer& bo = net->bufs[op.cd.out_buf];
      h_kind[i] = (op.fused_skip && net->use_tc) ? 4 : (op.plan && net->use_tc) ? 1 : 0;
      h_flops[i] = 2.0 * N * bo.H * bo.W * (double)op.cd.R * op.cd.S * op.cd.Cin * op.cd.Cout;
      if (h_geom) {
        int* g = h_geom + 8 * i;
        g[0] = bo.H; g[1] = bo.W; g[2] = op.cd.Cin; g[3] = op.cd.Cout; g[4] = op.cd.R; g[5] = op.cd.stride;
        g[6] = op.cd.res_buf >= 0; g[7] = op.plan ? tc_conv_plan_block_n(op.plan) : 0;
      }
    } else if (op.kind == 1 || op.kind == 3) {
      h_kind[i] = 2;
      h_flops[i] = 0.0;
      if (h_geom) {
        const NetBuffer& bo = net->bufs[op.out_buf];
        int* g = h_geom + 8 * i;
        g[0] = bo.H; g[1] = bo.W; g[2] = bo.C; g[3] = bo.C; g[4] = op.kind == 1 ? op.k : 0; g[5] = op.kind == 1 ? op.stride : 1; g[6] = 0; g[7] = 0;
      }
    } else {
      h_kind[i] = 3;
      h_flops[i] = 2.0 * N * (double)op.fc_cin * op.fc_cout;
      if (h_geom) {
        int* g = h_geom + 8 * i;
        g[0] = 1; g[1] = 1; g[2] = op.fc_cin; g[3] = op.fc_cout; g[4] = 1; g[5] = 1; g[6] = 0; g[7] = 0;
      }
    }
  }
  *num_ops = nops;
  for (auto& e : ev) cudaEventDestroy(e);
  cudaFree(d_logits);
  return rc;
}

int nib_net_forward_masked(nib_net* net, const nib_mask_args* args, float* d_logits, void* stream) {
  NIB_DEVICE_OR_FAIL();
  NIB_REQUIRE(net && net->finalized && args, "nib_net_forward_masked: bad handle/args");
  NIB_REQUIRE(args->N > 0 && args->N <= net->max_batch, "nib_net_forward_masked: N=%d outside (0, max_batch=%d]",
              args->N, net->max_batch);
  const NetBuffer& bi = net->bufs[net->input_buf];
  NIB_REQUIRE(args->H == bi.H && args->W == bi.W && args->C <= bi.C, "nib_net_forward_masked: image %dx%dx%d does not match the network input %dx%dx%d",
              args->C, args->H, args->W, bi.C, bi.H, bi.W);
  nib_mask_args a = *args;
  a.d_out = bi.ptr;
  a.out_dtype = net->bf16 ? NIB_BF16 : NIB_F32;
  a.layout = NIB_NHWC;
  a.c_stride = bi.C;
  a.pad_h = a.pad_w = bi.pad;
  int rc = mask_synth_impl(&a, (cudaStream_t)stream, true, net->dyn_n);
  net->launches += 1;
  if (rc != NIB_OK) return rc;
  return nib_net_forward(net, bi.ptr, NIB_IN_NATIVE, args->N, d_logits, stream);
}

int nib_net_buffer_info(nib_net* net, int buf, void** d_ptr, int* H, int* W, int* C, int* pad, int* dtype) {
  NIB_REQUIRE(net && buf >= 0 && buf < (int)net->bufs.size(), "nib_net_buffer_info: bad buffer id");
  const NetBuffer& b = net->bufs[buf];
  if (d_ptr) *d_ptr = b.ptr;
  if (H) *H = b.H;
  if (W) *W = b.W;
  if (C) *C = b.C;
  if (pad) *pad = b.pad;
  if (dtype) *dtype = b.kind == BUF_F32 ? NIB_F32 : b.kind == BUF_BF16 ? NIB_BF16 : 2 ;
  return NIB_OK;
}

int nib_net_read_buffer_nchw(nib_net* net, int buf, int N, float* d_out, void* stream) {
  NIB_DEVICE_OR_FAIL();
  NIB_REQUIRE(net && buf >= 0 && buf < (int)net->bufs.size() && d_out, "nib_net_read_buffer_nchw: bad arguments");
  NIB_REQUIRE(N > 0 && N <= net->max_batch, "nib_net_read_buffer_nchw: bad N");
  const NetBuffer& b = net->bufs[buf];
  NIB_REQUIRE(b.kind != BUF_SPLIT, "nib_net_read_buffer_nchw: convert a split buffer to fp32 first (nib_net_add_convert)");
  return launch_nhwc_to_nchw(b.ptr, N, b.C, b.H, b.W, b.C, b.pad, b.kind == BUF_BF16, d_out, (cudaStream_t)stream);
}

int nib_net_launch_counts(nib_net* net, long long* total, long long* tcgen05) {
  NIB_REQUIRE(net != nullptr, "nib_net_launch_counts: null handle");
  if (total) *total = net->launches;
  if (tcgen05) *tcgen05 = net->tc_launches;
  return NIB_OK;
}

int nib_net_set_tensor_core(nib_net* net, int enable) {
  NIB_REQUIRE(net != nullptr, "nib_net_set_tensor_core: null handle");
  NIB_REQUIRE(enable || !net->split, "nib_net_set_tensor_core: split-bf16 tensors exist only on the tensor path");
  net->use_tc = enable != 0;
  for (auto& g : net->graphs) cudaGraphExecDestroy(g.second.exec);
  net->graphs.clear();
  return NIB_OK;
// ... 19 lines not shown
```

Baseline: 44610.

## Fuse stem 7x7 conv with 3x3/2 max pool in a tcgen05 kernel

Result: faster. 45770 (median of 6 runs) (+2.6%).

```diff
diff --git a/include/nib.h b/include/nib.h
--- a/include/nib.h
+++ b/include/nib.h
@@ -80,7 +80,8 @@
 
 enum nib_conv_flags {
   NIB_CONV_RELU = 1,
-  NIB_CONV_PRE_BNRELU = 2
+  NIB_CONV_PRE_BNRELU = 2,
+  NIB_CONV_MAXPOOL3S2 = 4
 };
 
 typedef struct nib_conv_desc {
diff --git a/network_interpretation_imagenet_b200/_lib.py b/network_interpretation_imagenet_b200/_lib.py
--- a/network_interpretation_imagenet_b200/_lib.py
+++ b/network_interpretation_imagenet_b200/_lib.py
@@ -12,7 +12,7 @@
 F32, BF16 = 0, 1
 NCHW, NHWC = 0, 1
 PREC_FP32, PREC_BF16, PREC_X3, PREC_SPLIT = 0, 1, 2, 3
-CONV_RELU, CONV_PRE_BNRELU = 1, 2
+CONV_RELU, CONV_PRE_BNRELU, CONV_MAXPOOL3S2 = 1, 2, 4
 POOL_MAX, POOL_AVG = 0, 1
 IN_NCHW_F32, IN_NATIVE = 0, 1
 
diff --git a/network_interpretation_imagenet_b200/classifier.py b/network_interpretation_imagenet_b200/classifier.py
--- a/network_interpretation_imagenet_b200/classifier.py
+++ b/network_interpretation_imagenet_b200/classifier.py
@@ -58,14 +58,15 @@
         self.free.setdefault(self.shapes[b], []).append(b)
 
     def conv(self, in_buf, Cin, out_buf, Cout, w, b, k, stride, pad, relu, in_coff=0, out_coff=0, res=None, res_C=0,
-             pre=None):
+             pre=None, maxpool=False):
         d = _lib.ConvDesc()
         d.in_buf, d.in_coff, d.Cin = in_buf, in_coff, Cin
         d.out_buf, d.out_coff, d.Cout = out_buf, out_coff, Cout
         d.res_buf, d.res_coff, d.res_C = (res if res is not None else -1), 0, res_C
         d.R = d.S = k
         d.stride, d.pad = stride, pad
-        d.flags = (_lib.CONV_RELU if relu else 0) | (_lib.CONV_PRE_BNRELU if pre is not None else 0)
+        d.flags = ((_lib.CONV_RELU if relu else 0) | (_lib.CONV_PRE_BNRELU if pre is not None else 0)
+                   | (_lib.CONV_MAXPOOL3S2 if maxpool else 0))
         wn = _f32(w)
         bn_ = _f32(b) if b is not None else None
         ps = _f32(pre[0]) if pre is not None else None
@@ -244,6 +245,18 @@
     return 4 if Cin <= 4 else Cin
 
 
+def _pair(v):
+    return tuple(v) if isinstance(v, (tuple, list)) else (v, v)
+
+
+def _stem_pool_fused(conv, pool, in_cpix, W) -> bool:
+    if in_cpix != 4 or conv.out_channels != 64 or not isinstance(pool, nn.MaxPool2d):
+        return False
+    if (_pair(pool.kernel_size), _pair(pool.stride), _pair(pool.padding), _pair(pool.dilation)) != ((3, 3), (2, 2), (1, 1), (1, 1)):
+        return False
+    return not pool.ceil_mode and W % 2 == 0 and _out_hw(W, 7, 2, 3) <= 128
+
+
 def _lower_tv_resnet(m, hw, prec, precision, max_batch):
     H, W = hw
     b = _Builder(prec, max_batch)
@@ -254,15 +267,19 @@
     x_in = (b.buffer(H, W, 4 if cin <= 4 else 8, pad=3, pooled=False) if stem_tc
             else b.buffer(H, W, _in_cpad(cin), pooled=False, f32=split))
     Hc, Wc = _out_hw(H, c1.kernel_size[0], c1.stride[0], c1.padding[0]), _out_hw(W, c1.kernel_size[0], c1.stride[0], c1.padding[0])
-    t = b.buffer(Hc, Wc, c1.out_channels, f32=split)
     w, bias = fold_bn(c1.weight, c1.bias, m.bn1)
-    b.conv(x_in, cin, t, c1.out_channels, w, bias, c1.kernel_size[0], c1.stride[0], c1.padding[0], relu=True)
     mp = m.maxpool
     k, s, p = mp.kernel_size, mp.stride, mp.padding
     Hp, Wp = _out_hw(Hc, k, s, p), _out_hw(Wc, k, s, p)
-    x = b.buffer(Hp, Wp, c1.out_channels, f32=split)
-    b.pool(_lib.POOL_MAX, t, c1.out_channels, x, k, s, p)
-    b.release(t)
+    if stem_tc and _stem_pool_fused(c1, mp, 4 if cin <= 4 else 8, W):
+        x = b.buffer(Hp, Wp, c1.out_channels)
+        b.conv(x_in, cin, x, c1.out_channels, w, bias, 7, 2, 3, relu=True, maxpool=True)
+    else:
+        t = b.buffer(Hc, Wc, c1.out_channels, f32=split)
+        b.conv(x_in, cin, t, c1.out_channels, w, bias, c1.kernel_size[0], c1.stride[0], c1.padding[0], relu=True)
+        x = b.buffer(Hp, Wp, c1.out_channels, f32=split)
+        b.pool(_lib.POOL_MAX, t, c1.out_channels, x, k, s, p)
+        b.release(t)
     if split:
         xs = b.buffer(Hp, Wp, c1.out_channels)
         b.convert(x, xs)
@@ -429,9 +446,12 @@
     stem_tc = (precision == "bf16" and c0.kernel_size == (7, 7) and c0.stride == (2, 2) and c0.padding == (3, 3))
     x_in = b.buffer(H, W, 4, pad=3, pooled=False) if stem_tc else b.buffer(H, W, _in_cpad(3), pooled=False)
     Hc, Wc = _out_hw(H, 7, 2, 3), _out_hw(W, 7, 2, 3)
-    t = b.buffer(Hc, Wc, c0.out_channels)
     w, bias = fold_bn(c0.weight, None, f.norm0)
-    b.conv(x_in, 3, t, c0.out_channels, w, bias, 7, 2, 3, relu=True)
+    fused = stem_tc and _stem_pool_fused(c0, f.pool0, 4, W)
+    t = None
+    if not fused:
+        t = b.buffer(Hc, Wc, c0.out_channels)
+        b.conv(x_in, 3, t, c0.out_channels, w, bias, 7, 2, 3, relu=True)
     Hx, Wx = _out_hw(Hc, 3, 2, 1), _out_hw(Wc, 3, 2, 1)
     blocks = [getattr(f, n) for n in ("denseblock1", "denseblock2", "denseblock3", "denseblock4")]
     trans = [getattr(f, n) for n in ("transition1", "transition2", "transition3")]
@@ -442,7 +462,9 @@
         growth = layers[0].conv2.out_channels
         Ctot = Cin + growth * len(layers)
         buf = b.buffer(Hx, Wx, Ctot, pooled=False)
-        if prev_is_stem:
+        if prev_is_stem and fused:
+            b.conv(x_in, 3, buf, c0.out_channels, w, bias, 7, 2, 3, relu=True, maxpool=True)
+        elif prev_is_stem:
             b.pool(_lib.POOL_MAX, prev, Cin, buf, 3, 2, 1)
             b.release(prev)
         else:
diff --git a/network_interpretation_imagenet_b200/csrc/conv_tc.cu b/network_interpretation_imagenet_b200/csrc/conv_tc.cu
--- a/network_interpretation_imagenet_b200/csrc/conv_tc.cu
+++ b/network_interpretation_imagenet_b200/csrc/conv_tc.cu
@@ -518,6 +518,20 @@
   return (1u << 4) | (1u << 7) | (1u << 10) | ((uint32_t)(BLOCK_N >> 3) << 17) | ((uint32_t)(256 >> 4) << 24);
 }
 
+__device__ __forceinline__ void raw_rows_mma(uint32_t d_tmem, uint32_t a_addr, uint32_t b_base, uint32_t bh_bytes,
+                                             int raw_rows, int row_bytes, uint32_t lbo, uint32_t sbo, uint32_t idesc) {
+#pragma unroll 1
+  for (int r = 0; r < raw_rows; ++r) {
+    const uint32_t b_addr = b_base + (uint32_t)(r >> 1) * bh_bytes + (uint32_t)(r & 1) * (bh_bytes / 2);
+#pragma unroll
+    for (int ks = 0; ks < 2; ++ks) {
+      const uint64_t adesc = make_smem_desc_nosw(a_addr + (uint32_t)(r * row_bytes) + ks * 32, lbo, sbo);
+      const uint64_t bdesc = make_smem_desc_sw64(b_addr + ks * 32);
+      umma2_bf16(d_tmem, adesc, bdesc, idesc, (r | ks) != 0);
+    }
+  }
+}
+
 template <int BLOCK_N, int STAGES, bool HAS_RES, bool BRES, bool SPLIT = false>
 __global__ void __cluster_dims__(2, 1, 1) __launch_bounds__(TC3_THREADS_XF, 1)
 conv_tc3_kernel(const __grid_constant__ CUtensorMap tmA, const __grid_constant__ CUtensorMap tmB,
@@ -794,16 +808,8 @@
             const int q0 = ((tile / p.n_tiles) % p.col_tiles) * p.tile_rows;
             const uint32_t a_addr = smem_base + stage * SM::STAGE_BYTES + 16u * (uint32_t)q0;
             const uint32_t lbo = p.halo_swap ? 128u : 16u, sbo = p.halo_swap ? 16u : 128u;
-#pragma unroll 1
-            for (int r = 0; r < p.raw_rows; ++r) {
-              const uint32_t b_addr = smem_base + SM::BRES_OFFSET + (r >> 1) * SM::BH_BYTES + (r & 1) * (SM::BH_BYTES / 2);
-#pragma unroll
-              for (int ks = 0; ks < 2; ++ks) {
-                const uint64_t adesc = make_smem_desc_nosw(a_addr + (uint32_t)(r * p.halo_wp) + ks * 32, lbo, sbo);
-                const uint64_t bdesc = make_smem_desc_sw64(b_addr + ks * 32);
-                umma2_bf16(d_tmem, adesc, bdesc, idesc, (r | ks) != 0);
-              }
-            }
+            raw_rows_mma(d_tmem, a_addr, smem_base + SM::BRES_OFFSET, (uint32_t)SM::BH_BYTES, p.raw_rows, p.halo_wp, lbo, sbo,
+                         idesc);
             umma2_commit_both(empty_bar(stage));
             umma2_commit_both(tmem_full_bar(ab));
           }
@@ -1111,6 +1117,258 @@
 }
 
 
+static constexpr int SP_STAGES = 8;
+static constexpr int SP_SLOTS = 8;
+static constexpr int SP_THREADS = 64 + 256;
+struct SpSmem {
+  static constexpr int A_BYTES = TC_BLOCK_M * TC_BLOCK_K * 2;
+  static constexpr int BH_BYTES = 32 * TC_BLOCK_K * 2;
+  static constexpr int BRES_OFFSET = SP_STAGES * A_BYTES;
+  static constexpr int XBUF_OFFSET = BRES_OFFSET + 4 * BH_BYTES;
+  static constexpr int STG_OFFSET = XBUF_OFFSET + 2 * 2 * 4 * 128;
+  static constexpr int STG_BYTES = 16 * 64;
+  static constexpr int BIAS_OFFSET = STG_OFFSET + 8 * 2 * STG_BYTES;
+  static constexpr int BAR_OFFSET = BIAS_OFFSET + 64 * 4;
+  static constexpr int NUM_BARS = 2 * SP_STAGES + 2 * SP_SLOTS + 1;
+  static constexpr int TOTAL = BAR_OFFSET + NUM_BARS * 8 + 16;
+};
+
+struct StemPoolParams {
+  const float* bias;
+  int N;
+  int P, Q, PP, QP;
+  long long rows_total;
+  int out_coff;
+  int relu;
+  int row_bytes;
+  int a_bytes;
+  unsigned int* err_flag;
+};
+
+__device__ __forceinline__ void sp_rows(const StemPoolParams& p, long long g, long long g0, int& ip, int& pr, int& r_lo,
+                                        int& r_new, int& r_hi) {
+  ip = (int)(g / p.PP);
+  pr = (int)(g - (long long)ip * p.PP);
+  r_lo = max(2 * pr - 1, 0);
+  r_new = (g == g0 || pr == 0) ? r_lo : 2 * pr;
+  r_hi = min(2 * pr + 1, p.P - 1);
+}
+
+__global__ void __cluster_dims__(2, 1, 1) __launch_bounds__(SP_THREADS, 1)
+conv_stem_pool_kernel(const __grid_constant__ CUtensorMap tmA, const __grid_constant__ CUtensorMap tmB,
+                      const __grid_constant__ CUtensorMap tmOut, const __grid_constant__ CUtensorMap tmOutTail,
+                      const StemPoolParams p) {
+  using SM = SpSmem;
+  extern __shared__ __align__(1024) uint8_t smem_raw[];
+  const uint32_t smem_base = smem_u32(smem_raw);
+  if ((smem_base & 1023u) != 0) {
+    if (threadIdx.x == 0 && p.err_flag) atomicExch(p.err_flag, 9u);
+    __trap();
+  }
+  const uint32_t bar_base = smem_base + SM::BAR_OFFSET;
+  auto full_bar = [&](int s) { return bar_base + 8u * s; };
+  auto empty_bar = [&](int s) { return bar_base + 8u * (SP_STAGES + s); };
+  auto tmem_full_bar = [&](int s) { return bar_base + 8u * (2 * SP_STAGES + s); };
+  auto tmem_empty_bar = [&](int s) { return bar_base + 8u * (2 * SP_STAGES + SP_SLOTS + s); };
+  const uint32_t bres_full_bar = bar_base + 8u * (2 * SP_STAGES + 2 * SP_SLOTS);
+  const uint32_t tmem_slot = bar_base + 8u * SM::NUM_BARS;
+  uint32_t* tmem_slot_ptr = reinterpret_cast<uint32_t*>(smem_raw + (tmem_slot - smem_base));
+  float* bias_s = reinterpret_cast<float*>(smem_raw + SM::BIAS_OFFSET);
+
+  const int warp = threadIdx.x >> 5;
+  const int lane = threadIdx.x & 31;
+  const uint32_t rank = cluster_ctarank();
+  const int pair = blockIdx.x >> 1;
+  const int npairs = gridDim.x >> 1;
+  const long long g0 = p.rows_total * pair / npairs, g1 = p.rows_total * (pair + 1) / npairs;
+  constexpr uint32_t TMEM_COLS = SP_SLOTS * 64;
+
+  if (warp == 0 && lane == 0) {
+    prefetch_tmap(&tmA);
+    prefetch_tmap(&tmB);
+    prefetch_tmap(&tmOut);
+    prefetch_tmap(&tmOutTail);
+    for (int s = 0; s < SP_STAGES; ++s) {
+      mbar_init(full_bar(s), 1);
+      mbar_init(empty_bar(s), 1);
+    }
+    for (int s = 0; s < SP_SLOTS; ++s) {
+      mbar_init(tmem_full_bar(s), 1);
+      mbar_init(tmem_empty_bar(s), 16);
+    }
+    mbar_init(bres_full_bar, 1);
+    asm volatile("fence.mbarrier_init.release.cluster;" ::: "memory");
+  }
+  if (warp == 1) {
+    asm volatile("tcgen05.alloc.cta_group::2.sync.aligned.shared::cta.b32 [%0], %1;" ::"r"(tmem_slot), "r"(TMEM_COLS) : "memory");
+    asm volatile("tcgen05.relinquish_alloc_permit.cta_group::2.sync.aligned;" ::: "memory");
+  }
+  if (threadIdx.x >= 64 && threadIdx.x < 128) bias_s[threadIdx.x - 64] = p.bias ? __ldg(p.bias + threadIdx.x - 64) : 0.f;
+  tc_fence_before();
+  __syncthreads();
+  cluster_sync_all();
+  tc_fence_after();
+  const uint32_t tmem_base = *tmem_slot_ptr;
+  asm volatile("griddepcontrol.wait;" ::: "memory");
+  asm volatile("griddepcontrol.launch_dependents;" ::: "memory");
+
+  if (warp == 0) {
+    const uint32_t lbar0 = mapa_shared(full_bar(0), 0);
+    if (elect_one()) {
+      const uint32_t lb = mapa_shared(bres_full_bar, 0);
+      if (rank == 0) mbar_arrive_expect_tx(bres_full_bar, (uint32_t)(2 * 4 * SM::BH_BYTES));
+      for (int kb = 0; kb < 4; ++kb) {
+        const uint32_t dst = smem_base + SM::BRES_OFFSET + kb * SM::BH_BYTES;
+        tma2_load_2d(dst, &tmB, lb, kb * TC_BLOCK_K, (int)rank * 32);
+        tma2_load_2d(dst + SM::BH_BYTES / 2, &tmB, lb, kb * TC_BLOCK_K + 32, (int)rank * 32);
+      }
+    }
+    __syncwarp();
+    int k = 0;
+    for (long long g = g0; g < g1; ++g) {
+      int ip, pr, r_lo, r_new, r_hi;
+      sp_rows(p, g, g0, ip, pr, r_lo, r_new, r_hi);
+      for (int r = r_new; r <= r_hi; ++r, ++k) {
+        const int stage = k % SP_STAGES;
+        mbar_wait(empty_bar(stage), (uint32_t)(((k / SP_STAGES) & 1) ^ 1), p.err_flag, 1);
+        if (elect_one()) {
+          if (rank == 0) mbar_arrive_expect_tx(full_bar(stage), (uint32_t)(2 * p.a_bytes));
+          tma2_load_4d(smem_base + stage * SM::A_BYTES, &tmA, lbar0 + 8u * stage, 0, 0, 2 * r, 2 * ip + (int)rank);
+        }
+        __syncwarp();
+      }
+    }
+  } else if (warp == 1) {
+    if (rank == 0) {
+      constexpr uint32_t idesc = make_idesc_bf16_pair<64>();
+      mbar_wait(bres_full_bar, 0, p.err_flag, 7);
+      int k = 0;
+      for (long long g = g0; g < g1; ++g) {
+        int ip, pr, r_lo, r_new, r_hi;
+        sp_rows(p, g, g0, ip, pr, r_lo, r_new, r_hi);
+        for (int r = r_new; r <= r_hi; ++r, ++k) {
+          const int slot = k % SP_SLOTS, stage = k % SP_STAGES;
+          mbar_wait(tmem_empty_bar(slot), (uint32_t)(((k / SP_SLOTS) & 1) ^ 1), p.err_flag, 5);
+          mbar_wait(full_bar(stage), (uint32_t)((k / SP_STAGES) & 1), p.err_flag, 2);
+          tc_fence_after();
+          if (elect_one()) {
+            raw_rows_mma(tmem_base + (uint32_t)(slot * 64), smem_base + stage * SM::A_BYTES, smem_base + SM::BRES_OFFSET,
+                         (uint32_t)SM::BH_BYTES, 7, p.row_bytes, 16u, 128u, idesc);
+            umma2_commit_both(empty_bar(stage));
+            umma2_commit_both(tmem_full_bar(slot));
+          }
+          __syncwarp();
+        }
+      }
+    }
+  } else {
+    const int ew = warp - 2;
+    const int g = ew >> 2;
+    const int quarter = warp & 3;
+    const int col = quarter * 32 + lane;
+    const uint32_t lead_empty0 = mapa_shared(tmem_empty_bar(0), 0);
+    const uint32_t relu_floor = p.relu ? 0u : 0xFF80FF80u;
+    const bool has_bias = p.bias != nullptr;
+    const bool has_right = col + 1 < p.Q;
+    const bool emits = (lane & 1) == 0 && col < p.Q;
+    const int nq = min(16, p.QP - 16 * quarter);
+    const uint32_t xbuf = smem_base + SM::XBUF_OFFSET + (uint32_t)(g * 2 * 4 * 128);
+    const uint32_t bias_g = smem_u32(bias_s) + (uint32_t)(g * 32 * 4);
+    int k = 0, sbuf = 0;
+    for (long long gr = g0; gr < g1; ++gr, sbuf ^= 1) {
+      int ip, pr, r_lo, r_new, r_hi;
+      sp_rows(p, gr, g0, ip, pr, r_lo, r_new, r_hi);
+      const int img = 2 * ip + (int)rank;
+      auto slot_of = [&](int r) { return (r >= r_new ? k + (r - r_new) : k - 1) % SP_SLOTS; };
+      for (int r = r_new; r <= r_hi; ++r) {
+        const int kr = k + (r - r_new);
+        mbar_wait(tmem_full_bar(kr % SP_SLOTS), (uint32_t)((kr / SP_SLOTS) & 1), p.err_flag, 3);
+      }
+      tc_fence_after();
+      const uint32_t tl = tmem_base + ((uint32_t)(quarter * 32) << 16) + (uint32_t)(g * 32);
+      uint32_t v0[32], v1[32], v2[32];
+      tmem_ld_32x32b_x32(tl + (uint32_t)(slot_of(r_lo) * 64), v0);
+      tmem_ld_32x32b_x32(tl + (uint32_t)(slot_of(min(r_lo + 1, r_hi)) * 64), v1);
+      tmem_ld_32x32b_x32(tl + (uint32_t)(slot_of(min(r_lo + 2, r_hi)) * 64), v2);
+      tmem_ld_wait();
+      const bool carry = gr + 1 < g1 && pr + 1 < p.PP;
+      tc_fence_before();
+      __syncwarp();
+      if (lane == 0)
+        for (int r = r_lo; r <= r_hi - (carry ? 1 : 0); ++r) mbar_arrive_remote(lead_empty0 + 8u * (uint32_t)slot_of(r));
+      k += r_hi - r_new + 1;
+      float m[32];
+#pragma unroll
+      for (int j = 0; j < 32; ++j)
+        m[j] = fmaxf(fmaxf(__uint_as_float(v0[j]), __uint_as_float(v1[j])), __uint_as_float(v2[j]));
+      const uint32_t xb = xbuf + (uint32_t)(sbuf * 4 * 128);
+      if (lane == 31) {
+#pragma unroll
+        for (int j = 0; j < 8; ++j)
+          sts_v4(xb + (uint32_t)(quarter * 128 + j * 16), make_uint4(__float_as_uint(m[4 * j]), __float_as_uint(m[4 * j + 1]),
+                                                                     __float_as_uint(m[4 * j + 2]), __float_as_uint(m[4 * j + 3])));
+      }
+      float x[32];
+#pragma unroll
+      for (int j = 0; j < 32; ++j) {
+        const float rt = __shfl_down_sync(0xffffffffu, m[j], 1);
+        const float lf = __shfl_up_sync(0xffffffffu, m[j], 1);
+        x[j] = fmaxf(m[j], has_right ? rt : m[j]);
+        if (lane > 0) x[j] = fmaxf(x[j], lf);
+      }
+      named_bar_sync(1 + g, 128);
+      if (lane == 0 && quarter > 0) {
+#pragma unroll
+        for (int j = 0; j < 8; ++j) {
+          const uint4 u = lds_v4(xb + (uint32_t)((quarter - 1) * 128 + j * 16));
+          x[4 * j] = fmaxf(x[4 * j], __uint_as_float(u.x)); x[4 * j + 1] = fmaxf(x[4 * j + 1], __uint_as_float(u.y));
+          x[4 * j + 2] = fmaxf(x[4 * j + 2], __uint_as_float(u.z)); x[4 * j + 3] = fmaxf(x[4 * j + 3], __uint_as_float(u.w));
+        }
+      }
+      if (nq <= 0) continue;
+      const uint32_t stg = smem_base + SM::STG_OFFSET + (uint32_t)((ew * 2 + sbuf) * SM::STG_BYTES);
+      if (lane == 0) bulk_wait_read<1>();
+      __syncwarp();
+      if (emits) {
+#pragma unroll
+        for (int c = 0; c < 4; ++c) {
+          uint64_t a0 = pack_f32x2(__float_as_uint(x[8 * c + 0]), __float_as_uint(x[8 * c + 1]));
+          uint64_t a1 = pack_f32x2(__float_as_uint(x[8 * c + 2]), __float_as_uint(x[8 * c + 3]));
+          uint64_t a2 = pack_f32x2(__float_as_uint(x[8 * c + 4]), __float_as_uint(x[8 * c + 5]));
+          uint64_t a3 = pack_f32x2(__float_as_uint(x[8 * c + 6]), __float_as_uint(x[8 * c + 7]));
+          if (has_bias) {
+            const uint4 b0 = lds_v4(bias_g + (uint32_t)(c * 32)), b1 = lds_v4(bias_g + (uint32_t)(c * 32 + 16));
+            a0 = add_f32x2(a0, pack_f32x2(b0.x, b0.y)); a1 = add_f32x2(a1, pack_f32x2(b0.z, b0.w));
+            a2 = add_f32x2(a2, pack_f32x2(b1.x, b1.y)); a3 = add_f32x2(a3, pack_f32x2(b1.z, b1.w));
+          }
+          sts_v4(stg + (uint32_t)((lane >> 1) * 64 + c * 16),
+                 make_uint4(max_bf16x2(cvt_bf16x2(a0), relu_floor), max_bf16x2(cvt_bf16x2(a1), relu_floor),
+                            max_bf16x2(cvt_bf16x2(a2), relu_floor), max_bf16x2(cvt_bf16x2(a3), relu_floor)));
+        }
+      }
+      fence_async_smem();
+      __syncwarp();
+      if (lane == 0) {
+        if (img < p.N) {
+          const int row = (img * p.PP + pr) * p.QP + 16 * quarter;
+          if (nq == 16) tma_store_2d(&tmOut, stg, p.out_coff + 32 * g, row);
+          else tma_store_2d(&tmOutTail, stg, p.out_coff + 32 * g, row);
+        }
+        bulk_commit();
+      }
+    }
+    if (lane == 0) bulk_wait_read<0>();
+    tc_fence_before();
+  }
+  __syncthreads();
+  cluster_sync_all();
+  if (warp == 1) {
+    tc_fence_after();
+    asm volatile("tcgen05.dealloc.cta_group::2.sync.aligned.b32 %0, %1;" ::"r"(tmem_base), "r"(TMEM_COLS) : "memory");
+  }
+}
+
+
 struct TcFusedParams {
   const float* bias1;
   const float* bias2;
@@ -1510,6 +1768,7 @@
   int num_k_blocks, cblocks;
   int halo_wp, halo_r, halo_tpi, halo_cb, halo_n;
   int raw_rows, col_tiles;
+  int stem_pool;
   unsigned int* err_flag;
 };
 
@@ -1554,6 +1813,16 @@
   return 0;
 }
 
+static bool stem4_raw_rows_fit(const ConvParams& p) {
+  const int Wp = p.Win + 2 * p.in_halo;
+  return 6 * Wp * 8 + 16 * 127 + 64 <= TC_BLOCK_M * TC_BLOCK_K * 2 && raw_row_inner(Wp * 4) > 0;
+}
+
+bool tc_conv_is_stem_pool(const ConvParams& p) {
+  return p.pool_P > 0 && !p.split && tc_conv_is_stem4(p) && p.Cout == 64 && stem4_raw_rows_fit(p) &&
+         p.pool_P == (p.P - 1) / 2 + 1 && p.pool_Q == (p.Q - 1) / 2 + 1;
+}
+
 static int raw3x3_col_tiles(int Q) {
   if (Q <= TC_BLOCK_M) return 1;
   for (int t = 2; Q / t >= TC_BLOCK_M / 2; ++t)
@@ -1597,6 +1866,7 @@
 }
 
 bool tc_conv_supported(const ConvParams& p) {
+  if (p.pool_P > 0) return tc_conv_is_stem_pool(p);
   if (p.split) {
     if (p.Cin % TC_BLOCK_K != 0 || p.Cout % 64 != 0 || p.in_coff != 0 || p.out_coff != 0 || p.in_lo_off != p.Cin) return false;
     if (p.in_cstride != 2 * p.Cin || p.out_cstride < p.out_lo_off + p.Cout || p.out_lo_off % 64 != 0) return false;
@@ -1656,6 +1926,37 @@
   return NIB_OK;
 }
 
+static int encode_stem4_raw_rows(CUtensorMap* tm, const ConvParams& p, int max_batch) {
+  const int Hp = p.Hin + 6, Wp = p.Win + 6, inner = raw_row_inner(Wp * 4);
+  cuuint64_t dims[4] = {(cuuint64_t)inner, (cuuint64_t)(Wp * 4 / inner), (cuuint64_t)Hp, (cuuint64_t)max_batch};
+  cuuint64_t strides[3] = {(cuuint64_t)inner * 2, (cuuint64_t)Wp * 8, (cuuint64_t)Hp * Wp * 8};
+  cuuint32_t box[4] = {(cuuint32_t)inner, (cuuint32_t)(Wp * 4 / inner), 7, 1};
+  cuuint32_t es[4] = {1, 1, 1, 1};
+  CUresult r = g_encodeTiled(tm, CU_TENSOR_MAP_DATA_TYPE_BFLOAT16, 4, const_cast<void*>(p.in), dims, strides, box, es,
+                             CU_TENSOR_MAP_INTERLEAVE_NONE, CU_TENSOR_MAP_SWIZZLE_NONE, CU_TENSOR_MAP_L2_PROMOTION_L2_256B,
+                             CU_TENSOR_MAP_FLOAT_OOB_FILL_NONE);
+  if (r != CUDA_SUCCESS) {
+    set_error("cuTensorMapEncodeTiled (stem, raw rows) failed (%d)", (int)r);
+    return NIB_ECUDA;
+  }
+  return NIB_OK;
+}
+
+static int encode_stem4_weights(CUtensorMap* tm, const ConvParams& p, int rows) {
+  cuuint64_t dims[2] = {256, (cuuint64_t)p.Cout};
+  cuuint64_t strides[1] = {256 * 2};
+  cuuint32_t box[2] = {32, (cuuint32_t)rows};
+  cuuint32_t es[2] = {1, 1};
+  CUresult r = g_encodeTiled(tm, CU_TENSOR_MAP_DATA_TYPE_BFLOAT16, 2, const_cast<void*>(p.w_alt), dims, strides, box, es,
+                             CU_TENSOR_MAP_INTERLEAVE_NONE, CU_TENSOR_MAP_SWIZZLE_64B, CU_TENSOR_MAP_L2_PROMOTION_L2_256B,
+                             CU_TENSOR_MAP_FLOAT_OOB_FILL_NONE);
+  if (r != CUDA_SUCCESS) {
+    set_error("cuTensorMapEncodeTiled (stem weights, 64B swizzle) failed (%d)", (int)r);
+    return NIB_ECUDA;
+  }
+  return NIB_OK;
+}
+
 int tc_conv_plan_create(const ConvParams& p, int max_batch, TcConvPlan** out) {
   int rc = load_driver_fns();
   if (rc != NIB_OK) return rc;
@@ -1668,34 +1969,50 @@
   plan->err_flag = g_err_flag;
   plan->block_n = pick_block_n(p.Cout);
   plan->tile_rows = TC_BLOCK_M;
+  if (p.pool_P > 0) {
+    if (!tc_conv_is_stem_pool(p)) {
+      set_error("tc_conv_plan_create: the fused stem + max pool needs the 4-channel raw-row 7x7/2 stem with 64 outputs");
+      delete plan;
+      return NIB_EINVAL;
+    }
+    plan->stem_pool = 1;
+    plan->halo_wp = (p.Win + 6) * 8;
+    rc = encode_stem4_raw_rows(&plan->tmA, p, max_batch);
+    if (rc == NIB_OK) rc = encode_stem4_weights(&plan->tmBh, p, 32);
+    if (rc == NIB_OK) {
+      cuuint64_t dims[2] = {(cuuint64_t)p.out_cstride, (cuuint64_t)max_batch * p.pool_P * p.pool_Q};
+      cuuint64_t strides[1] = {(cuuint64_t)p.out_cstride * 2};
+      cuuint32_t es[2] = {1, 1};
+      for (int t = 0; t < 2 && rc == NIB_OK; ++t) {
+        cuuint32_t box[2] = {32, (cuuint32_t)(t == 1 && p.pool_Q % 16 ? p.pool_Q % 16 : 16)};
+        CUresult r = g_encodeTiled(t ? &plan->tmOutTail : &plan->tmOut, CU_TENSOR_MAP_DATA_TYPE_BFLOAT16, 2, p.out, dims,
+                                   strides, box, es, CU_TENSOR_MAP_INTERLEAVE_NONE, CU_TENSOR_MAP_SWIZZLE_NONE,
+                                   CU_TENSOR_MAP_L2_PROMOTION_L2_256B, CU_TENSOR_MAP_FLOAT_OOB_FILL_NONE);
+        if (r != CUDA_SUCCESS) {
+          set_error("cuTensorMapEncodeTiled (pooled stem pixels) failed (%d)", (int)r);
+          rc = NIB_ECUDA;
+        }
+      }
+    }
+    if (rc != NIB_OK) { delete plan; return rc; }
+    plan->v3 = 1;
+    *out = plan;
+    return NIB_OK;
+  }
   if (tc_conv_is_stem4(p)) {
     plan->im2col = 3;
     plan->cblocks = 1;
     plan->num_k_blocks = 4;
     plan->tile_rows = p.Q;
     const int Hp = p.Hin + 6, Wp = p.Win + 6;
-    int inner = 0;
-    {
-      static const bool off = getenv("NIB_TC_NO_HALO") != nullptr;
-      if (!off && 6 * Wp * 8 + 16 * 127 + 64 <= 16384) inner = raw_row_inner(Wp * 4);
-    }
-    if (inner > 0) {
+    static const bool no_halo = getenv("NIB_TC_NO_HALO") != nullptr;
+    if (!no_halo && stem4_raw_rows_fit(p)) {
       plan->im2col = 5;
       plan->raw_rows = 7;
       plan->col_tiles = 1;
       plan->halo_wp = Wp * 8;
-      cuuint64_t dims[4] = {(cuuint64_t)inner, (cuuint64_t)(Wp * 4 / inner), (cuuint64_t)Hp, (cuuint64_t)max_batch};
-      cuuint64_t strides[3] = {(cuuint64_t)inner * 2, (cuuint64_t)Wp * 8, (cuuint64_t)Hp * Wp * 8};
-      cuuint32_t box[4] = {(cuuint32_t)inner, (cuuint32_t)(Wp * 4 / inner), 7, 1};
-      cuuint32_t es[4] = {1, 1, 1, 1};
-      CUresult r = g_encodeTiled(&plan->tmA, CU_TENSOR_MAP_DATA_TYPE_BFLOAT16, 4, const_cast<void*>(p.in), dims, strides,
-                                 box, es, CU_TENSOR_MAP_INTERLEAVE_NONE, CU_TENSOR_MAP_SWIZZLE_NONE,
-                                 CU_TENSOR_MAP_L2_PROMOTION_L2_256B, CU_TENSOR_MAP_FLOAT_OOB_FILL_NONE);
-      if (r != CUDA_SUCCESS) {
-        set_error("cuTensorMapEncodeTiled (stem, raw rows) failed (%d)", (int)r);
-        delete plan;
-        return NIB_ECUDA;
-      }
+      rc = encode_stem4_raw_rows(&plan->tmA, p, max_batch);
+      if (rc != NIB_OK) { delete plan; return rc; }
     } else {
       cuuint64_t dims[4] = {32, (cuuint64_t)p.Q, (cuuint64_t)Hp, (cuuint64_t)max_batch};
       cuuint64_t strides[3] = {16, (cuuint64_t)Wp * 8, (cuuint64_t)Hp * Wp * 8};
@@ -1712,20 +2029,8 @@
     }
     rc = finish_plan(plan, p, max_batch, p.w_alt, 4 * 64);
     if (rc != NIB_OK) { delete plan; return rc; }
-    {
-      cuuint64_t dims[2] = {256, (cuuint64_t)p.Cout};
-      cuuint64_t strides[1] = {256 * 2};
-      cuuint32_t box[2] = {32, (cuuint32_t)(plan->block_n / 2)};
-      cuuint32_t es[2] = {1, 1};
-      CUresult r = g_encodeTiled(&plan->tmBh, CU_TENSOR_MAP_DATA_TYPE_BFLOAT16, 2, const_cast<void*>(p.w_alt), dims, strides,
-                                 box, es, CU_TENSOR_MAP_INTERLEAVE_NONE, CU_TENSOR_MAP_SWIZZLE_64B,
-                                 CU_TENSOR_MAP_L2_PROMOTION_L2_256B, CU_TENSOR_MAP_FLOAT_OOB_FILL_NONE);
-      if (r != CUDA_SUCCESS) {
-        set_error("cuTensorMapEncodeTiled (stem weights, 64B swizzle) failed (%d)", (int)r);
-        delete plan;
-        return NIB_ECUDA;
-      }
-    }
+    rc = encode_stem4_weights(&plan->tmBh, p, plan->block_n / 2);
+    if (rc != NIB_OK) { delete plan; return rc; }
     plan->tmB = plan->tmBh;
     *out = plan;
     return NIB_OK;
@@ -2154,7 +2459,48 @@
   return NIB_OK;
 }
 
+static int tc_stem_pool_launch(const TcConvPlan* plan, const ConvParams& p, cudaStream_t st) {
+  using SM = SpSmem;
+  static_assert(SM::TOTAL <= 232448, "exceeds the 227 KB per-CTA shared memory limit");
+  static bool attr_set = false;
+  if (!attr_set) {
+    NIB_CUDA(cudaFuncSetAttribute(conv_stem_pool_kernel, cudaFuncAttributeMaxDynamicSharedMemorySize, SM::TOTAL));
+    attr_set = true;
+  }
+  StemPoolParams kp;
+  memset(&kp, 0, sizeof(kp));
+  kp.bias = p.bias;
+  kp.N = p.M / (p.P * p.Q);
+  kp.P = p.P; kp.Q = p.Q; kp.PP = p.pool_P; kp.QP = p.pool_Q;
+  kp.rows_total = (long long)((kp.N + 1) / 2) * p.pool_P;
+  kp.out_coff = p.out_coff;
+  kp.relu = p.relu;
+  kp.row_bytes = plan->halo_wp;
+  kp.a_bytes = 7 * plan->halo_wp;
+  kp.err_flag = plan->err_flag;
+  if (kp.rows_total == 0) return NIB_OK;
+  const long long max_pairs = num_sms() / 2;
+  const int pairs = (int)(kp.rows_total < max_pairs ? kp.rows_total : max_pairs);
+  static const bool pdl = getenv("NIB_TC_NO_PDL") == nullptr;
+  cudaStreamCaptureStatus cap = cudaStreamCaptureStatusNone;
+  cudaStreamIsCapturing(st, &cap);
+  cudaLaunchConfig_t cfg;
+  memset(&cfg, 0, sizeof(cfg));
+  cfg.gridDim = dim3(2 * pairs);
+  cfg.blockDim = dim3(SP_THREADS);
+  cfg.dynamicSmemBytes = SM::TOTAL;
+  cfg.stream = st;
+  cudaLaunchAttribute attr[1];
+  attr[0].id = cudaLaunchAttributeProgrammaticStreamSerialization;
+  attr[0].val.programmaticStreamSerializationAllowed = 1;
+  cfg.attrs = attr;
+  cfg.numAttrs = (pdl && cap == cudaStreamCaptureStatusNone) ? 1 : 0;
+  NIB_CUDA(cudaLaunchKernelEx(&cfg, conv_stem_pool_kernel, plan->tmA, plan->tmBh, plan->tmOut, plan->tmOutTail, kp));
+  return NIB_OK;
+}
+
 int tc_conv_launch(const TcConvPlan* plan, const ConvParams& p, cudaStream_t st) {
+  if (plan->stem_pool) return tc_stem_pool_launch(plan, p, st);
   TcKernelParams kp;
   memset(&kp, 0, sizeof(kp));
   kp.bias = p.bias;
diff --git a/network_interpretation_imagenet_b200/csrc/layers.cuh b/network_interpretation_imagenet_b200/csrc/layers.cuh
--- a/network_interpretation_imagenet_b200/csrc/layers.cuh
+++ b/network_interpretation_imagenet_b200/csrc/layers.cuh
@@ -22,6 +22,7 @@
   const int* dyn_n;
   int split;
   int in_lo_off, out_lo_off, res_lo_off;
+  int pool_P, pool_Q;
 };
 
 struct PoolParams {
diff --git a/network_interpretation_imagenet_b200/csrc/net.cu b/network_interpretation_imagenet_b200/csrc/net.cu
--- a/network_interpretation_imagenet_b200/csrc/net.cu
+++ b/network_interpretation_imagenet_b200/csrc/net.cu
@@ -194,7 +194,17 @@
   NIB_REQUIRE(d->R > 0 && d->S > 0 && d->stride > 0 && d->pad >= 0, "nib_net_add_conv: bad filter geometry");
   const int P = (bi.H + 2 * d->pad - d->R) / d->stride + 1;
   const int Q = (bi.W + 2 * d->pad - d->S) / d->stride + 1;
-  NIB_REQUIRE(P == bo.H && Q == bo.W, "nib_net_add_conv: output buffer is %dx%d but conv produces %dx%d", bo.H, bo.W, P, Q);
+  if (d->flags & NIB_CONV_MAXPOOL3S2) {
+    NIB_REQUIRE(net->bf16 && d->R == 7 && d->S == 7 && d->stride == 2 && d->pad == 3 && d->Cin <= 4 && bi.C == 4 &&
+                    bi.pad == 3 && d->Cout == 64 && d->res_buf < 0 && !(d->flags & NIB_CONV_PRE_BNRELU),
+                "nib_net_add_conv: NIB_CONV_MAXPOOL3S2 needs a bf16 network's 7x7/2/3 stem on a 4-channel input with a "
+                "3-pixel halo, 64 outputs, no residual");
+    const int Pp = (P - 1) / 2 + 1, Qp = (Q - 1) / 2 + 1;
+    NIB_REQUIRE(Pp == bo.H && Qp == bo.W, "nib_net_add_conv: output buffer is %dx%d but conv + max pool produces %dx%d",
+                bo.H, bo.W, Pp, Qp);
+  } else {
+    NIB_REQUIRE(P == bo.H && Q == bo.W, "nib_net_add_conv: output buffer is %dx%d but conv produces %dx%d", bo.H, bo.W, P, Q);
+  }
   NIB_REQUIRE(bo.pad == 0, "nib_net_add_conv: output buffers with halo are not supported");
   if (d->res_buf >= 0) {
     const NetBuffer& br = net->bufs[d->res_buf];
@@ -420,6 +430,12 @@
   p->R = d.R; p->S = d.S; p->stride = d.stride; p->pad = d.pad;
   p->relu = (d.flags & NIB_CONV_RELU) ? 1 : 0;
   p->dyn_n = net->dyn_n;
+  if (d.flags & NIB_CONV_MAXPOOL3S2) {
+    p->pool_P = bo.H; p->pool_Q = bo.W;
+    p->P = (bi.H + 2 * d.pad - d.R) / d.stride + 1;
+    p->Q = (bi.W + 2 * d.pad - d.S) / d.stride + 1;
+    p->M = N * p->P * p->Q;
+  }
 }
 
 static void fill_xform_conv_params(const nib_net* net, const NetOp& op, int N, ConvParams* p) {
@@ -490,6 +506,12 @@
         continue;
       }
       fill_conv_params(net, op, net->max_batch, &p);
+      if (op.cd.flags & NIB_CONV_MAXPOOL3S2) {
+        NIB_REQUIRE(tc_conv_supported(p), "nib_net_finalize: the stem + max pool op needs an output width <= 128 (got %d)", p.Q);
+        int rc = tc_conv_plan_create(p, net->max_batch, &op.plan);
+        if (rc != NIB_OK) return rc;
+        continue;
+      }
       if (tc_conv_supported(p)) {
         int rc = tc_conv_plan_create(p, net->max_batch, &op.plan);
         if (rc != NIB_OK) {
@@ -549,7 +571,7 @@
         fill_packed_conv_params(net, op, N, &p);
         rc = tc_conv_launch(op.plan, p, st);
         net->tc_launches++;
-      } else if (op.plan && (net->use_tc || net->split)) {
+      } else if (op.plan && (net->use_tc || net->split || (op.cd.flags & NIB_CONV_MAXPOOL3S2))) {
         rc = tc_conv_launch(op.plan, p, st);
         net->tc_launches++;
       } else if (net->x3 && op.d_w_hi && conv_x3_supported(p)) {
@@ -692,8 +714,11 @@
     const NetOp& op = net->ops[i];
     if (op.kind == 0) {
       const NetBuffer& bo = net->bufs[op.cd.out_buf];
-      h_kind[i] = (op.fused_skip && net->use_tc) ? 4 : (op.plan && net->use_tc) ? 1 : 0;
-      h_flops[i] = 2.0 * N * bo.H * bo.W * (double)op.cd.R * op.cd.S * op.cd.Cin * op.cd.Cout;
+      const bool pooled = (op.cd.flags & NIB_CONV_MAXPOOL3S2) != 0;
+      h_kind[i] = (op.fused_skip && net->use_tc) ? 4 : (op.plan && (net->use_tc || pooled)) ? 1 : 0;
+      ConvParams cp;
+      fill_conv_params(net, op, N, &cp);
+      h_flops[i] = 2.0 * cp.M * (double)op.cd.R * op.cd.S * op.cd.Cin * op.cd.Cout;
       if (h_geom) {
         int* g = h_geom + 8 * i;
         g[0] = bo.H; g[1] = bo.W; g[2] = op.cd.Cin; g[3] = op.cd.Cout; g[4] = op.cd.R; g[5] = op.cd.stride;
```
